# bacpop/sparrowhawk

Measured on AMD Instinct MI355X. Metric: Gbases/s assembled, k=31 150bp reads, higher is better.
Workload: dtype u64

## Files before the change

### sparrowhawk_amd/csrc/count_part.h

```cpp
#pragma once
#include <hip/hip_runtime.h>
#include <stdint.h>
#include <type_traits>
#include "kmer.h"

namespace shk {

static constexpr int PART_THREADS = 1024;
static constexpr int COUNT_THREADS = 1024;
static constexpr int PART_MAX_P = 16384;

struct PartParams {
    uint32_t P, G, slice_cap;
    int k, m;
    uint32_t max_n;
};

template <int RW> struct Rec { uint64_t w[RW]; };

__device__ __forceinline__ uint64_t sel4(uint32_t b, uint64_t t0, uint64_t t1, uint64_t t2, uint64_t t3) {
    uint64_t lo = (b & 1) ? t1 : t0;
    uint64_t hi = (b & 1) ? t3 : t2;
    return (b & 2) ? hi : lo;
}
// ... 871 lines not shown
        if (threadIdx.x == 0) ctl.prog_den = R ? R : 1u;
        for (uint32_t r0 = w_begin; r0 < w_end; r0 += 64) {
            if (ctl.overflow || ctl.n_used > (S / 10) * 9) { atomicMax(&ctl.prog_num, min(R, (r0 - w_begin) * (COUNT_THREADS / 64) + 1u)); break; }
            Rec<RW> rec = nxt;
            const uint32_t n = have_nxt ? (uint32_t)(rec.w[RW - 1] >> 58) + 1u : 0u;
            if (n) rec_canonicalise<RW>(rec.w, n, k);
            const uint32_t wgt = w_nxt;
            nxt = nxt2; have_nxt = have_nxt2; w_nxt = w_nxt2;
            have_nxt2 = fetch(r0 + 128u + (uint32_t)lane, nxt2, w_nxt2);
            if (n && !rec_insert<W>(tb.rt, ctl, rec, wgt)) {
                if (ovf && mod == 1 && (r0 - w_begin) * 2u < (w_end - w_begin)) ctl.overflow = 1;
                else expand(rec, n, wgt);
            }
        }
        {
            constexpr uint32_t SRc = decltype(tb.rt)::SR;
            auto &rt = tb.rt;
            if (threadIdx.x < 64) rt.nhist[threadIdx.x] = 0;
            __syncthreads();
            for (uint32_t s = threadIdx.x; s < SRc; s += COUNT_THREADS)
                if (rt.rst[s] >= 3u) atomicAdd(&rt.nhist[(uint32_t)(rt.w[s][RW - 1] >> 58)], 1u);
            __syncthreads();
            if (threadIdx.x < 64) {
                const uint32_t v = rt.nhist[threadIdx.x];
                uint32_t incl = v;
                for (int o = 1; o < 64; o <<= 1) { const uint32_t u = __shfl_up(incl, o); if (lane >= o) incl += u; }
                rt.nbase[threadIdx.x] = incl - v;
                if (threadIdx.x == 63) ctl.n_recs = incl;
            }
            __syncthreads();
            for (uint32_t s = threadIdx.x; s < SRc; s += COUNT_THREADS)
                if (rt.rst[s] >= 3u) rt.order[atomicAdd(&rt.nbase[(uint32_t)(rt.w[s][RW - 1] >> 58)], 1u)] = (uint16_t)s;
            __syncthreads();
            const uint32_t n_recs = ctl.n_recs;
            if (threadIdx.x == 0 && ctl.prog_num == 0) ctl.prog_den = n_recs ? n_recs : 1u;
            __syncthreads();
            for (uint32_t i = threadIdx.x; i < n_recs; i += COUNT_THREADS) {
                if (ctl.overflow || ctl.n_used > (S / 10) * 9) { atomicMax(&ctl.prog_num, i - threadIdx.x + 1u); break; }
                const uint32_t s = rt.order[i];
                Rec<RW> rec;
#pragma unroll
                for (int o = 0; o < RW; o++) rec.w[o] = rt.w[s][o];
                expand(rec, (uint32_t)(rec.w[RW - 1] >> 58) + 1u, rt.rst[s] - 2u);
            }
        }
        __syncthreads();
        const bool over = ctl.overflow != 0 || ctl.n_used > (S / 10) * 9;
        if (over && ovf && mod == 1) {
            defer(mine, true);
            return;
        }
        if (over) {
            if (mod >= 4096 || ctl.sp + 1 > 16) { if (threadIdx.x == 0) flags[0] = 1; break; }
            __syncthreads();
            if (threadIdx.x == 0) {
                const uint32_t num = ctl.prog_num ? ctl.prog_num : ctl.prog_den;
                const double est = (double)ctl.n_used * (double)ctl.prog_den / (double)num;
                uint32_t factor = 2;
                while ((double)factor * (0.6 * S) < est && mod * factor < 4096u) factor <<= 1;
                ctl.st_res[ctl.sp] = res; ctl.st_step[ctl.sp] = mod; ctl.st_factor[ctl.sp] = factor; ctl.st_next[ctl.sp] = 0;
                ctl.sp += 1;
            }
            continue;
        }
        static_assert(2u * decltype(tb.rt)::SR >= S, "emit list");
        table_emit<W>(tb, ctl, mine, threshold, histo, out_keys, out_cnt, out_cap, out_cursor, reinterpret_cast<uint16_t *>(tb.rt.rst), whist);
    }
    if (threadIdx.x == 0 && ovf && defer_after) atomicAdd(&ovf_n[1], 1u);
   }();
  }
    __syncthreads();
    for (uint32_t b = threadIdx.x; b < 500; b += COUNT_THREADS)
        if (whist[b]) atomicAdd(&histo[b], (unsigned long long)whist[b]);
    if (threadIdx.x == 0 && ctl.n_inst) atomicAdd(n_inst, ctl.n_inst);
}


template <int W> struct DedupeShared {
    RecTable<W, (W == 1 ? 3072u : ((69632u / (16u * W + 6u)) & ~63u))> rt;
};
template <int W>
__global__ __launch_bounds__(COUNT_THREADS, W <= 2 ? 8 : 4) void k_dedupe_partitions(
                                                                     RunView rvw, uint32_t p_first, uint32_t n_parts,
                                                                     const unsigned long long *__restrict__ base,
                                                                     uint64_t *__restrict__ out_recs, uint32_t *__restrict__ out_w,
                                                                     uint32_t *__restrict__ n_out, uint32_t *__restrict__ work_counter,
                                                                     OvfRec *__restrict__ ovf , uint32_t *__restrict__ ovf_n,
                                                                     uint32_t defer_after, uint32_t kmer_cap,
                                                                     uint32_t *__restrict__ verdict_out ) {
    constexpr int RW = 2 * W;
    __shared__ DedupeShared<W> tb;
    __shared__ CountCtl ctl;
    __shared__ uint32_t wtot[4];
    constexpr uint32_t SR = decltype(tb.rt)::SR;
    const int lane = threadIdx.x & 63;
    const int k = rvw.k;
    const uint32_t S_runs = rvw.S;
    const uint32_t n_here = n_parts - p_first;
    __shared__ uint32_t forced_sh;
    if (threadIdx.x == 0) forced_sh = 0;
    __syncthreads();
    bool forced = false;
    uint32_t pi_next = 0;
    for (uint32_t pi = blockIdx.x; pi < n_here; pi = pi_next) {
        const uint32_t p = p_first + pi;
        uint32_t f = 0; unsigned long long addr = 0;
        if (threadIdx.x < S_runs) { f = rvw.run_cnt[(uint64_t)p * S_runs + threadIdx.x]; addr = rvw.run_addr16[(uint64_t)p * S_runs + threadIdx.x]; }
        forced = forced_sh != 0;
        if (forced) {
            unsigned long long inst = 0;
            const uint64_t *src = reinterpret_cast<const uint64_t *>(addr << 4);
            for (uint32_t i = 0; i < f; i++) inst += (src[(uint64_t)i * RW + RW - 1] >> 58) + 1ull;
            __syncthreads();
            if (threadIdx.x == 0) { ctl.part_inst = 0; ctl.next_pi = gridDim.x + atomicAdd(work_counter, 1u); }
            __syncthreads();
            for (int o = 32; o > 0; o >>= 1) inst += __shfl_down(inst, o);
            if (lane == 0 && inst) atomicAdd(&ctl.part_inst, inst);
            __syncthreads();
            pi_next = ctl.next_pi;
            if (threadIdx.x == 0) {
                n_out[p] = 0;
                if (ctl.part_inst) { const uint32_t slot = atomicAdd(ovf_n, 1u); OvfRec o; o.p = p; o.est_distinct = 0u; o.instances = ctl.part_inst; ovf[slot] = o; }
            }
            continue;
        }
        uint32_t incl = f;
        if (threadIdx.x < 256) {
            for (int o = 1; o < 64; o <<= 1) { const uint32_t v = __shfl_up(incl, o); if (lane >= o) incl += v; }
            if (lane == 63) wtot[threadIdx.x >> 6] = incl;
        }
        __syncthreads();
        if (threadIdx.x < 256) {
            uint32_t off = 0;
            for (uint32_t w = 0; w < (threadIdx.x >> 6); w++) off += wtot[w];
            if (threadIdx.x < S_runs) { ctl.pre[threadIdx.x] = off + incl - f; ctl.roff[threadIdx.x] = addr; }
        }
        if (threadIdx.x == 0) {
            ctl.pre[S_runs] = wtot[0] + wtot[1] + wtot[2] + wtot[3];
            ctl.rec_used = 0; ctl.n_emit = 0; ctl.part_inst = 0;
            ctl.next_pi = gridDim.x + atomicAdd(work_counter, 1u);
        }
        for (uint32_t s = threadIdx.x; s < SR; s += COUNT_THREADS) tb.rt.rst[s] = 0;
        __syncthreads();
        pi_next = ctl.next_pi;
        const uint32_t R = ctl.pre[S_runs];
        auto hand_over = [&]() {
            unsigned long long inst = 0;
            const uint32_t pw = (((R + (COUNT_THREADS / 64) - 1) / (COUNT_THREADS / 64)) + 63u) & ~63u;
            const uint32_t wb = min(R, (threadIdx.x >> 6) * pw), we = min(R, wb + pw);
            uint32_t lo = 0, hi = S_runs;
            { const uint32_t r = min(wb + (uint32_t)lane, R ? R - 1u : 0u);
              while (hi - lo > 1) { const uint32_t mid = (lo + hi) >> 1; if (ctl.pre[mid] <= r) lo = mid; else hi = mid; } }
            uint32_t nx = ctl.pre[lo + 1];
            for (uint32_t r = wb + (uint32_t)lane; r < we; r += 64) {
                while (r >= nx) { lo++; nx = ctl.pre[lo + 1]; }
                const uint64_t *src = reinterpret_cast<const uint64_t *>(ctl.roff[lo] << 4) + (uint64_t)(r - ctl.pre[lo]) * RW;
                inst += (src[RW - 1] >> 58) + 1ull;
            }
            for (int o = 32; o > 0; o >>= 1) inst += __shfl_down(inst, o);
            if (lane == 0 && inst) atomicAdd(&ctl.part_inst, inst);
            __syncthreads();
            if (threadIdx.x == 0) {
                n_out[p] = 0;
                if (R) { const uint32_t slot = atomicAdd(ovf_n, 1u); OvfRec o; o.p = p; o.est_distinct = 0u; o.instances = ctl.part_inst; ovf[slot] = o; }
            }
        };
        uint64_t *dst = out_recs + base[p] * RW;
        uint32_t *dst_w = out_w + base[p];
        const uint32_t per_wave = (((R + (COUNT_THREADS / 64) - 1) / (COUNT_THREADS / 64)) + 63u) & ~63u;
        const uint32_t w_begin = min(R, (threadIdx.x >> 6) * per_wave), w_end = min(R, w_begin + per_wave);
        uint32_t run_lo = 0, run_next = 0;
        {
            uint32_t lo = 0, hi = S_runs;
            const uint32_t r = min(w_begin + (uint32_t)lane, R ? R - 1u : 0u);
            while (hi - lo > 1) { const uint32_t mid = (lo + hi) >> 1; if (ctl.pre[mid] <= r) lo = mid; else hi = mid; }
            run_lo = lo; run_next = ctl.pre[lo + 1];
        }
        auto fetch = [&](uint32_t r, Rec<RW> &rec) -> uint32_t {
            if (r >= w_end) return 0u;
            while (r >= run_next) { run_lo++; run_next = ctl.pre[run_lo + 1]; }
            const uint64_t *src = reinterpret_cast<const uint64_t *>(ctl.roff[run_lo] << 4) + (uint64_t)(r - ctl.pre[run_lo]) * RW;
#pragma unroll
            for (int o = 0; o < RW; o += 2) {
                const ulonglong2 v2 = *reinterpret_cast<const ulonglong2 *>(src + o);
                rec.w[o] = v2.x; rec.w[o + 1] = v2.y;
            }
            return 1u;
        };
        Rec<RW> nxt, nxt2;
#pragma unroll
        for (int o = 0; o < RW; o++) { nxt.w[o] = 0; nxt2.w[o] = 0; }
        uint32_t have_nxt = fetch(w_begin + (uint32_t)lane, nxt);
        uint32_t have_nxt2 = fetch(w_begin + 64u + (uint32_t)lane, nxt2);
        for (uint32_t r0 = w_begin; r0 < w_end; r0 += 64) {
            Rec<RW> rec = nxt;
            const uint32_t n = have_nxt ? (uint32_t)(rec.w[RW - 1] >> 58) + 1u : 0u;
            if (n) rec_canonicalise<RW>(rec.w, n, k);
            nxt = nxt2; have_nxt = have_nxt2;
            have_nxt2 = fetch(r0 + 128u + (uint32_t)lane, nxt2);
            const bool pass = n && !rec_insert<W>(tb.rt, ctl, rec);
            const unsigned long long m = __ballot(pass);
            if (m) {
                uint32_t at = 0;
                if (lane == (int)__builtin_ctzll(m)) at = atomicAdd(&ctl.n_emit, (uint32_t)__popcll(m));
                at = __shfl(at, (int)__builtin_ctzll(m)) + (uint32_t)__popcll(m & ((1ull << lane) - 1ull));
                if (pass) { part_store_record<RW>(rec.w, dst + (uint64_t)at * RW); dst_w[at] = 1u; }
            }
        }
        auto &rt = tb.rt;
        if (threadIdx.x < 64) rt.nhist[threadIdx.x] = 0;
        __syncthreads();
        for (uint32_t s = threadIdx.x; s < SR; s += COUNT_THREADS)
            if (rt.rst[s] >= 3u) atomicAdd(&rt.nhist[(uint32_t)(rt.w[s][RW - 1] >> 58)], 1u);
        __syncthreads();
        const uint32_t n_pass = ctl.n_emit;
        if (threadIdx.x < 64) {
            const uint32_t v = rt.nhist[threadIdx.x];
            uint32_t incl2 = v;
            for (int o = 1; o < 64; o <<= 1) { const uint32_t u = __shfl_up(incl2, o); if (lane >= o) incl2 += u; }
            rt.nbase[threadIdx.x] = n_pass + incl2 - v;
            if (threadIdx.x == 63) ctl.n_recs = n_pass + incl2;
        }
        __syncthreads();
        const bool hand = ovf && (ctl.n_recs > kmer_cap || (R > kmer_cap / 4u && 2u * ctl.n_recs > R));
        if (ovf && threadIdx.x == 0 && R) {
            const uint32_t add = hand ? 0x10001u : 1u;
            const uint32_t x = atomicAdd(&ovf_n[1], add) + add;
            const uint32_t n_over = x >> 16, n_tried = x & 0xFFFFu;
            if (defer_after && n_over >= defer_after && 2u * n_over >= n_tried) {
                forced_sh = 1u;
                if (verdict_out) atomicOr(verdict_out, 0x80000000u);
            }
        }
        if (hand) { hand_over(); continue; }
        for (uint32_t s = threadIdx.x; s < SR; s += COUNT_THREADS) {
            const uint32_t st = rt.rst[s];
            if (st < 3u) continue;
            const uint32_t at = atomicAdd(&rt.nbase[(uint32_t)(rt.w[s][RW - 1] >> 58)], 1u);
            uint64_t r[RW];
#pragma unroll
            for (int o = 0; o < RW; o++) r[o] = rt.w[s][o];
            part_store_record<RW>(r, dst + (uint64_t)at * RW);
            dst_w[at] = st - 2u;
        }
        __syncthreads();
        if (threadIdx.x == 0) n_out[p] = ctl.n_recs;
    }
}

template <int W>
__global__ __launch_bounds__(COUNT_THREADS, W <= 2 ? 8 : 4) void k_count_weighted(
    const uint64_t *__restrict__ recs, const uint32_t *__restrict__ weights, const unsigned long long *__restrict__ base,
    const uint32_t *__restrict__ n_recs, uint32_t p_first, uint32_t n_parts, uint32_t merge , int k, uint32_t threshold,
    unsigned long long *__restrict__ histo, KeyArr<W> out_keys, uint32_t *__restrict__ out_cnt,
    unsigned long long out_cap, unsigned long long *__restrict__ out_cursor,
    unsigned long long *__restrict__ n_inst, OvfRec *__restrict__ ovf, uint32_t *__restrict__ ovf_n,
    unsigned long long *__restrict__ work_and_tally ,
    uint32_t probe_groups, uint32_t defer_after,
    EmitRanges er ) {
    constexpr int RW = 2 * W;
    constexpr uint32_t S = KmerTable<W>::S;
    __shared__ KmerTable<W> tb;
    __shared__ CountCtlCore ctl;
    constexpr uint32_t ELIST = W == 1 ? S : 64;
    __shared__ uint16_t elist[ELIST];
    __shared__ uint32_t whist[500];
    __shared__ uint32_t next_g_sh, force_sh;
    const int lane = threadIdx.x & 63;
    for (uint32_t b = threadIdx.x; b < 500; b += COUNT_THREADS) whist[b] = 0;
    if (threadIdx.x == 0) ctl.n_inst = 0;
    const uint32_t n_groups = (n_parts + merge - 1) / merge;
    unsigned long long mine = 0;
    auto count_range = [&](const uint32_t (&pm)[4], uint32_t nm) -> bool {
        uint32_t Rj[4]; unsigned long long bj[4]; uint32_t Rt = 0;
#pragma unroll
        for (int j = 0; j < 4; j++) {
            const bool in = (uint32_t)j < nm;
            Rj[j] = in ? n_recs[pm[j]] : 0u; bj[j] = in ? base[pm[j]] : 0ull;
            Rt += Rj[j];
        }
        auto fetch = [&](uint32_t r, Rec<RW> &rec, uint32_t &wgt) {
            if (r < Rt) {
                unsigned long long at = bj[0] + r;
                uint32_t pre = Rj[0];
#pragma unroll
                for (int j = 1; j < 4; j++) { if (r >= pre) at = bj[j] + (r - pre); pre += Rj[j]; }
                const uint64_t *src = recs + at * RW;
#pragma unroll
                for (int o = 0; o < RW; o += 2) {
                    const ulonglong2 v2 = *reinterpret_cast<const ulonglong2 *>(src + o);
                    rec.w[o] = v2.x; rec.w[o + 1] = v2.y;
                }
                wgt = weights[at];
            }
        };
        Rec<RW> nxt; uint32_t w_nxt = 0;
#pragma unroll
        for (int o = 0; o < RW; o++) nxt.w[o] = 0;
        fetch(threadIdx.x, nxt, w_nxt);
        __syncthreads();
        if (threadIdx.x == 0) {
            ctl.n_used = 0; ctl.overflow = 0; ctl.n_emit = 0; ctl.wave_cursor = 0; ctl.rec_used = 0;
            ctl.prog_num = 0; ctl.prog_den = Rt ? Rt : 1u;
        }
        kmer_table_reset<W>(tb, ctl);
        mine = 0;
        for (uint32_t r0 = 0; r0 < Rt; r0 += COUNT_THREADS) {
            if (ctl.overflow || ctl.n_used > (S / 10) * 9) break;
            Rec<RW> rec = nxt; const uint32_t weight = w_nxt;
            const uint32_t r = r0 + threadIdx.x;
            fetch(r + COUNT_THREADS, nxt, w_nxt);
            if (r >= Rt) continue;
            const uint32_t n = (uint32_t)(rec.w[RW - 1] >> 58) + 1u;
            Kmer<W> f = km_zero<W>();
            for (uint32_t s = 0; s < n; s++) {
                if (ctl.overflow || ctl.n_used > (S / 10) * 9) break;
                if (s) {
#pragma unroll
                    for (int o = 0; o < RW - 1; o++) rec.w[o] = (rec.w[o] >> 2) | (rec.w[o + 1] << 62);
                    rec.w[RW - 1] >>= 2;
                }
                Kmer<W> rv;
#pragma unroll
                for (int j = 0; j < W; j++) rv.w[j] = ~rec.w[j];
                rv.w[W - 1] &= km_topmask<W>(k);
                if (s) km_push_back<W>(f, (uint32_t)(rec.w[W - 1] >> ((2 * (k - 1)) & 63)) & 3u, k);
                else f = km_revcomp<W>(rv, k);
                const bool use_r = km_less<W>(rv, f);
                Kmer<W> c;
#pragma unroll
                for (int j = 0; j < W; j++) c.w[j] = use_r ? rv.w[j] : f.w[j];
                const uint32_t h = km_mix32<W>(c);
                if (!lds_insert<W>(tb, ctl, c, h ^ __builtin_amdgcn_alignbit(h, h, 19), weight, true)) ctl.overflow = 1;
                mine += weight;
            }
        }
        __syncthreads();
        return !(ctl.overflow != 0 || ctl.n_used > (S / 10) * 9);
    };
    auto emit = [&](uint32_t er_g) {
        if constexpr (W == 1) table_emit<W>(tb, ctl, mine, threshold, histo, out_keys, out_cnt, out_cap, out_cursor, elist, whist, 0u, er, er_g);
        else table_emit<W>(tb, ctl, mine, threshold, histo, out_keys, out_cnt, out_cap, out_cursor, tb.state, whist, 0u, er, er_g);
    };
    auto mark_broken = [&]() { if (threadIdx.x == 0 && er.broken) *er.broken = 1u; };
    uint32_t *const tally = reinterpret_cast<uint32_t *>(work_and_tally) + 1;
    bool in_sample = true;
    auto defer = [&](uint32_t p, bool was_tried) {
        const uint32_t R = n_recs[p];
        const uint64_t *src = recs + base[p] * RW;
        const uint32_t *src_w = weights + base[p];
        mark_broken();
        __syncthreads();
        if (threadIdx.x == 0) { ctl.tried = 0; ctl.part_inst = 0; }
        __syncthreads();
        unsigned long long m = was_tried ? mine : 0ull;
        for (int o = 32; o > 0; o >>= 1) m += __shfl_down(m, o);
        if (lane == 0 && m) atomicAdd(&ctl.tried, m);
        unsigned long long inst = 0;
        for (uint32_t r = threadIdx.x; r < R; r += COUNT_THREADS)
            inst += ((src[(uint64_t)r * RW + RW - 1] >> 58) + 1ull) * (unsigned long long)src_w[r];
        for (int o = 32; o > 0; o >>= 1) inst += __shfl_down(inst, o);
        if (lane == 0 && inst) atomicAdd(&ctl.part_inst, inst);
        __syncthreads();
        if (threadIdx.x == 0 && R) {
            const double est = ctl.tried ? (double)ctl.n_used * (double)ctl.part_inst / (double)ctl.tried : (double)ctl.part_inst;
            const uint32_t slot = atomicAdd(ovf_n, 1u);
            OvfRec o; o.p = p; o.est_distinct = !was_tried ? 0u  : est > 4.0e9 ? 0xFFFFFFFFu : est < 1.0 ? 1u : (uint32_t)est; o.instances = ctl.part_inst;
            ovf[slot] = o;
        }
        if (threadIdx.x == 0 && was_tried && defer_after && in_sample) atomicAdd(tally, 0x10001u);
    };
    uint32_t g_next = 0;
    for (uint32_t g = blockIdx.x; g < n_groups; in_sample = false, g = g_next) {
        uint32_t pm[4] = {0, 0, 0, 0}, nm = 0;
#pragma unroll
        for (uint32_t j = 0; j < 4; j++) {
            const uint32_t pj = g + j * n_groups;
            const bool v = j < merge && pj < n_parts && pj >= p_first;
#pragma unroll
            for (uint32_t q = 0; q < 4; q++) if (v && nm == q) pm[q] = pj;
            nm += v ? 1u : 0u;
        }
        __syncthreads();
        if (threadIdx.x == 0) {
            const unsigned long long wt = atomicAdd(work_and_tally, 1ull);
            const uint32_t x = (uint32_t)(wt >> 32), n_over = x >> 16, n_tried = x & 0xFFFFu;
            next_g_sh = gridDim.x + (uint32_t)wt;
            force_sh = (defer_after && g >= probe_groups && n_over >= defer_after && 4u * n_over >= 3u * n_tried) ? 1u : 0u;
        }
        __syncthreads();
        g_next = next_g_sh;
        if (nm == 0) continue;
        if (force_sh) {
#pragma unroll
            for (uint32_t j = 0; j < 4; j++) if (j < nm) defer(pm[j], false);
            continue;
        }
        if (nm > 1 && count_range(pm, nm)) {
            emit(g);
            if (threadIdx.x == 0 && defer_after && in_sample) atomicAdd(tally, nm);
            continue;
        }
        if (nm > 1) mark_broken();
#pragma unroll
        for (uint32_t j = 0; j < 4; j++) {
            if (j >= nm) continue;
            const uint32_t one[4] = {pm[j], 0, 0, 0};
            if (count_range(one, 1u)) { emit(nm == 1 ? g : 0xFFFFFFFFu); if (threadIdx.x == 0 && defer_after && in_sample) atomicAdd(tally, 1u); }
            else defer(pm[j], true);
        }
    }
    __syncthreads();
    for (uint32_t b = threadIdx.x; b < 500; b += COUNT_THREADS)
        if (whist[b]) atomicAdd(&histo[b], (unsigned long long)whist[b]);
    if (threadIdx.x == 0 && ctl.n_inst) atomicAdd(n_inst, ctl.n_inst);
}

template <int RW>
__global__ __launch_bounds__(256) void k_pack_dedup(const uint64_t *__restrict__ src, const uint32_t *__restrict__ src_w,
                                                    const unsigned long long *__restrict__ src_base, const uint32_t *__restrict__ n_out,
                                                    const unsigned long long *__restrict__ dst_base,
                                                    uint64_t *__restrict__ dst, uint32_t *__restrict__ dst_w) {
    const uint32_t p = blockIdx.x, R = n_out[p];
    const uint64_t *sp = src + src_base[p] * RW;
    uint64_t *dp = dst + dst_base[p] * RW;
    for (uint32_t r = threadIdx.x; r < R; r += blockDim.x) {
#pragma unroll
        for (int o = 0; o < RW; o += 2)
            *reinterpret_cast<ulonglong2 *>(dp + (uint64_t)r * RW + o) = *reinterpret_cast<const ulonglong2 *>(sp + (uint64_t)r * RW + o);
        dst_w[dst_base[p] + r] = src_w[src_base[p] + r];
    }
}

// ... 267 lines not shown
```

### sparrowhawk_amd/csrc/ctl_words.h

```cpp
#pragma once
#include <stddef.h>
#include <stdint.h>

namespace shk {

static constexpr int CTL_WORDS = 32;

struct CountWords {
    union { unsigned long long row_cursor;
            unsigned long long g_instances; };
    union { unsigned long long instances;
            unsigned long long g_overflow; };
    uint32_t part_too_large, bucket_splits;
    uint32_t n_handed_over, tally;
    unsigned long long bucket_list_len;
    unsigned long long spare5[3];
    uint32_t p1_spare, p1_seg_too_long;
    union { unsigned long long p1_max_fill;
            unsigned long long bloom_keys; };
    unsigned long long spare10;
    unsigned long long probe_work;
    unsigned long long dedupe_work;
    unsigned long long spare13;
    uint32_t groups_out, group_tally;
    unsigned long long spare15[7];
    unsigned long long er_cursor;
    unsigned long long er_broken;
    unsigned long long spare24[8];
};
static inline unsigned tally_tried(uint32_t t) { return t & 0xFFFFu; }
static inline unsigned tally_over(uint32_t t) { return t >> 16; }
static inline unsigned long long er_rows(unsigned long long cursor) { return cursor >> 32; }

struct GraphWords {
    unsigned long long spare0;
    unsigned long long table_flag;
    unsigned long long slots_used;
    unsigned long long n_cand, n_tips;
    union { unsigned long long tips_removed;
            unsigned long long n_splitters; };
    union { unsigned long long bubbles_removed;
            unsigned long long n_chains; };
    unsigned long long n_ring_splitters;
    uint32_t collapse_flag, n_spl_wanted;
    unsigned long long n_alive;
    unsigned long long n_walked;
    unsigned long long spare11[2];
    union { unsigned long long xq_count;
            unsigned long long halflink_flags; };
    unsigned long long writer_flag;
    unsigned long long spare15;
    unsigned long long r0_tips_removed, r0_bubbles_removed;
    unsigned long long plan_state, plan_bytes, plan_emitted;
    unsigned long long spare21[11];
};

#define SHK_CTL_AT(S, m, slot, half) static_assert(offsetof(S, m) == (slot) * 8 + (half) * 4, #S "::" #m " moved")
static_assert(sizeof(CountWords) == CTL_WORDS * 8 && sizeof(GraphWords) == CTL_WORDS * 8, "32 control words");
SHK_CTL_AT(CountWords, row_cursor, 0, 0);     SHK_CTL_AT(CountWords, g_instances, 0, 0);
SHK_CTL_AT(CountWords, instances, 1, 0);      SHK_CTL_AT(CountWords, g_overflow, 1, 0);
SHK_CTL_AT(CountWords, part_too_large, 2, 0); SHK_CTL_AT(CountWords, bucket_splits, 2, 1);
SHK_CTL_AT(CountWords, n_handed_over, 3, 0);  SHK_CTL_AT(CountWords, tally, 3, 1);
SHK_CTL_AT(CountWords, bucket_list_len, 4, 0);
SHK_CTL_AT(CountWords, p1_spare, 8, 0);       SHK_CTL_AT(CountWords, p1_seg_too_long, 8, 1);
SHK_CTL_AT(CountWords, p1_max_fill, 9, 0);    SHK_CTL_AT(CountWords, bloom_keys, 9, 0);
SHK_CTL_AT(CountWords, probe_work, 11, 0);    SHK_CTL_AT(CountWords, dedupe_work, 12, 0);
SHK_CTL_AT(CountWords, groups_out, 14, 0);    SHK_CTL_AT(CountWords, group_tally, 14, 1);
SHK_CTL_AT(CountWords, er_cursor, 22, 0);     SHK_CTL_AT(CountWords, er_broken, 23, 0);
SHK_CTL_AT(GraphWords, spare0, 0, 0);         SHK_CTL_AT(GraphWords, table_flag, 1, 0);
SHK_CTL_AT(GraphWords, slots_used, 2, 0);     SHK_CTL_AT(GraphWords, n_cand, 3, 0);
SHK_CTL_AT(GraphWords, n_tips, 4, 0);
SHK_CTL_AT(GraphWords, tips_removed, 5, 0);   SHK_CTL_AT(GraphWords, n_splitters, 5, 0);
SHK_CTL_AT(GraphWords, bubbles_removed, 6, 0); SHK_CTL_AT(GraphWords, n_chains, 6, 0);
SHK_CTL_AT(GraphWords, n_ring_splitters, 7, 0);
SHK_CTL_AT(GraphWords, collapse_flag, 8, 0);  SHK_CTL_AT(GraphWords, n_spl_wanted, 8, 1);
SHK_CTL_AT(GraphWords, n_alive, 9, 0);        SHK_CTL_AT(GraphWords, n_walked, 10, 0);
SHK_CTL_AT(GraphWords, xq_count, 13, 0);      SHK_CTL_AT(GraphWords, halflink_flags, 13, 0);
SHK_CTL_AT(GraphWords, writer_flag, 14, 0);
SHK_CTL_AT(GraphWords, r0_tips_removed, 16, 0); SHK_CTL_AT(GraphWords, r0_bubbles_removed, 17, 0);
SHK_CTL_AT(GraphWords, plan_state, 18, 0);    SHK_CTL_AT(GraphWords, plan_bytes, 19, 0);
SHK_CTL_AT(GraphWords, plan_emitted, 20, 0);
#undef SHK_CTL_AT

}
```

### sparrowhawk_amd/csrc/pipeline.h

```cpp
#pragma once
#include <stdint.h>
#include <string>
#include <vector>
#include <map>
#include <memory>

namespace shk {

struct ShardComm;

class TextArrival {
public:
    virtual ~TextArrival() {}
    virtual const char *base() const = 0;
    virtual size_t total() const = 0;
    virtual void wait_range(size_t begin, size_t end) = 0;
    void wait_all() { wait_range(0, total()); }
    virtual int finish(std::string &err) = 0;
};

struct RawContig {
    const char *ext = nullptr; size_t ext_n = 0;
    std::string own;
    uint64_t kc = 0;
    const char *head = nullptr, *tail = nullptr; uint32_t ends_n = 0;
    const char *data() const { return ext ? ext : own.data(); }
    size_t size() const { return ext ? ext_n : own.size(); }
};

struct StageTimes {
    std::map<std::string, double> ms;
    void add(const std::string &k, double v) { ms[k] += v; }
};

struct DevPiece { const uint32_t *d_bases, *d_seg_off; uint64_t n_seg, n_bases; };

class IPipeline {
public:
    virtual ~IPipeline() {}
    virtual int count_batch(const uint32_t *d_bases, const uint32_t *d_seg_off, uint64_t n_seg,
                            uint64_t n_bases, std::string &err) = 0;
    virtual int count_batch_host(uint32_t *d_bases, uint32_t *d_seg_off, const uint32_t *h_bases, const uint32_t *h_seg_off,
                                 uint64_t n_seg, uint64_t n_bases, std::string &err) = 0;
    virtual int count_batch_pieces(const DevPiece *pieces, size_t n_pieces, std::string &err) = 0;
    virtual void expect_more_batches() = 0;
    virtual void set_bloom(bool on) = 0;
    virtual void set_verbose(bool on) = 0;
    virtual void single_batch_resident(bool on) = 0;
    virtual int histogram(uint64_t histo[500], uint32_t emit_threshold, std::string &err) = 0;
    virtual int filter(uint32_t threshold, std::string &err) = 0;
    virtual uint64_t total_instances() const = 0;
    virtual uint64_t n_distinct() const = 0;
    virtual uint64_t n_solid() const = 0;
    virtual int get_distinct(uint64_t *keys, uint32_t *counts, uint64_t cap, std::string &err) = 0;
    virtual int get_solid(uint64_t *keys, uint32_t *counts, uint64_t cap, std::string &err) = 0;
    virtual int build_graph(std::string &err) = 0;
    virtual int correct(bool tips, bool bubbles, std::string &err) = 0;
    virtual int collapse(std::vector<RawContig> &out, std::string &err, const char **json = nullptr, size_t *json_len = nullptr,
                         uint64_t *n_contigs = nullptr, TextArrival **arrival = nullptr) = 0;
    virtual int get_adjacency(uint8_t *adj_initial, uint8_t *adj_final, uint8_t *alive,
                              uint64_t cap, std::string &err) = 0;
    virtual int shard_partition(const uint32_t *d_bases, const uint32_t *d_seg_off, uint64_t n_seg, uint64_t n_bases,
                                uint32_t n_partitions, std::vector<uint64_t> &part_records, std::string &err) = 0;
    virtual uint32_t rec_words() const = 0;
    virtual int shard_pack(void *d_send, const uint64_t *base_records, uint32_t n_partitions, std::string &err) = 0;
    virtual int shard_dedupe(std::vector<uint64_t> &part_records, std::string &err) = 0;
    virtual int shard_pack_dedup(void *d_send, void *d_send_w, const uint64_t *base_records, uint32_t n_partitions, std::string &err) = 0;
    virtual void shard_drop_dedup() = 0;
    virtual int shard_count(const void *d_recv, const void *d_recv_w , const uint64_t *run_off, const uint32_t *run_cnt,
                            uint32_t n_owned, uint32_t n_sources, uint32_t emit_threshold, uint64_t histo[500], std::string &err) = 0;
    virtual int shard_rows(uint32_t threshold, const void **keys_soa, const void **cnt, uint64_t *n, std::string &err) = 0;
    virtual int shard_set_solid(const void *const *keys_soa, const void *cnt, uint64_t n, const uint64_t histo[500],
                                uint64_t total_instances, std::string &err) = 0;
    virtual int shard_keep_local(uint32_t world, uint32_t rank, uint32_t n_count_partitions, const uint64_t *rows_per_rank,
                                 const uint64_t histo[500], uint64_t total_instances, std::string &err) = 0;
    virtual bool sharded_graph() const = 0;
    virtual uint64_t n_solid_global() const = 0;
    virtual int shard_assemble(ShardComm *comm, bool tips, bool bubbles, std::vector<RawContig> &out, std::string &err) = 0;
    virtual StageTimes &times() = 0;
    virtual void drain() = 0;
    virtual void *stream() = 0;
    virtual int device() const = 0;
};

class DeferScope {
public:
    explicit DeferScope(IPipeline *pipe);
    ~DeferScope();
    DeferScope(const DeferScope &) = delete;
    DeferScope &operator=(const DeferScope &) = delete;
private:
    IPipeline *pipe_; void *list_; void *prev_;
};

IPipeline *make_pipeline(int k, std::string &err);
int device_count();
int current_device();
int set_device(int dev);

int host_canonical(const char *seq, uint32_t k, uint64_t *out_words, int *orient);
uint64_t host_nthash(const char *seq, uint32_t k);

int device_upload(const void *host, size_t bytes, void **dptr, std::string &err);
void device_free(void *dptr);
void device_pool_trim();
void *device_pool_alloc(size_t &bytes);
int stream_read_gbs(size_t bytes, int iters, double *gbs, std::string &err);
void device_pool_release(void *p, size_t bytes);
std::shared_ptr<void> mem_acct_new();
std::shared_ptr<void> mem_acct_set(std::shared_ptr<void> a);
uint64_t mem_acct_peak(const std::shared_ptr<void> &a);
uint64_t mem_acct_current(const std::shared_ptr<void> &a);
void mem_acct_replay(const int64_t *deltas, size_t n, uint64_t *peak, uint64_t *current);
int device_stream_sync(void *stream, std::string &err);
int device_copy_h2d_async(void *dst, const void *src, size_t bytes, void *stream, std::string &err);
int device_download(void *host, const void *dptr, size_t bytes, std::string &err);

}
```

### sparrowhawk_amd/csrc/pipeline.hip

```cpp
#include <hip/hip_runtime.h>
#include <hipcub/hipcub.hpp>
#include <thread>
#include <stdint.h>
#include <stdio.h>
#include <stdlib.h>
#include <string.h>
#include <algorithm>
#include <atomic>
#include <chrono>
#include <map>
#include <memory>
#include <mutex>
#include <string>
#include <vector>

#include "ctl_words.h"
#include "kmer.h"
#include "pipeline.h"
#include "shard_comm.h"
#include "unitig_graph.h"
#include "unitig_graph_gpu.h"

namespace shk {

// ... 203 lines not shown
}

static std::mutex g_stream_mu;
static std::multimap<int, hipStream_t> &stream_cache() { static auto *c = new std::multimap<int, hipStream_t>(); return *c; }
static hipStream_t stream_pool_get(int dev) {
    std::lock_guard<std::mutex> lk(g_stream_mu);
    auto it = stream_cache().find(dev);
    if (it == stream_cache().end()) return nullptr;
    hipStream_t s = it->second; stream_cache().erase(it); return s;
}
static void stream_pool_put(int dev, hipStream_t s) {
    {
        std::lock_guard<std::mutex> lk(g_stream_mu);
        if (stream_cache().size() < 32) { stream_cache().emplace(dev, s); return; }
    }
    (void)hipStreamDestroy(s);
}

static std::mutex &upload_token(int dev) { static std::mutex m[16]; return m[(unsigned)dev % 16u]; }

static inline int grid_for(uint64_t work, int block = 256, int max_blocks = 256 * 16) {
    uint64_t b = (work + block - 1) / block;
    if (b < 1) b = 1;
    if (b > (uint64_t)max_blocks) b = max_blocks;
    return (int)b;
}

static inline hipError_t stream_wait(hipStream_t s) {
    static const bool blocking = getenv("SHK_BLOCKING_SYNC") != nullptr;
    if (blocking) return hipStreamSynchronize(s);
    const auto t0 = std::chrono::steady_clock::now();
    for (;;) {
        const hipError_t e = hipStreamQuery(s);
        if (e != hipErrorNotReady) return e;
        if (std::chrono::steady_clock::now() - t0 > std::chrono::milliseconds(5)) return hipStreamSynchronize(s);
    }
}

struct EvTimer {
    hipEvent_t a, b; hipStream_t st; bool ok = false;
    explicit EvTimer(hipStream_t s, bool on = true) : st(s) {
        if (!on) return;
        ok = hipEventCreate(&a) == hipSuccess && hipEventCreate(&b) == hipSuccess;
        if (ok) (void)hipEventRecord(a, st);
    }
    bool on() const { return ok; }
    double stop() {
        if (!ok) return 0.0;
        (void)hipEventRecord(b, st); (void)hipEventSynchronize(b);
        float ms = 0; (void)hipEventElapsedTime(&ms, a, b);
        return ms;
    }
    ~EvTimer() { if (ok) { (void)hipEventDestroy(a); (void)hipEventDestroy(b); } }
    void mark() { if (ok) (void)hipEventRecord(b, st); }
    double elapsed() {
        if (!ok) return 0.0;
        (void)hipEventSynchronize(b);
        float ms = 0; (void)hipEventElapsedTime(&ms, a, b);
        return ms;
    }
    struct Pending { std::string name; hipEvent_t a, b; };
    void stop_later(const char *name, std::vector<Pending> &pending) {
        if (!ok) return;
        (void)hipEventRecord(b, st);
        pending.push_back(Pending{name, a, b});
        ok = false;
    }
    static void resolve(std::vector<Pending> &pending, StageTimes &times) {
        for (auto &p : pending) {
            (void)hipEventSynchronize(p.b);
            float ms = 0; (void)hipEventElapsedTime(&ms, p.a, p.b);
            times.add(p.name, ms);
            (void)hipEventDestroy(p.a); (void)hipEventDestroy(p.b);
        }
        pending.clear();
    }
};

static inline uint64_t env_u64(const char *name, uint64_t dflt) {
    const char *v = getenv(name);
    return (v && *v) ? strtoull(v, nullptr, 10) : dflt;
}

__global__ __launch_bounds__(256) void k_fill2(uint32_t *a, unsigned long long na, uint32_t va, uint32_t *b, unsigned long long nb, uint32_t vb) {
    const unsigned long long stride = (unsigned long long)gridDim.x * blockDim.x;
    for (unsigned long long i = (unsigned long long)blockIdx.x * blockDim.x + threadIdx.x; i < na + nb; i += stride) {
        if (i < na) a[i] = va; else b[i - na] = vb;
    }
}
__global__ __launch_bounds__(256) void k_stride_fill(unsigned long long *out, uint32_t n, unsigned long long stride) {
    for (uint32_t i = blockIdx.x * blockDim.x + threadIdx.x; i < n; i += gridDim.x * blockDim.x) out[i] = (unsigned long long)i * stride;
}
static inline hipError_t fill2_async(void *a, size_t bytes_a, uint32_t va, void *b, size_t bytes_b, uint32_t vb, hipStream_t st) {
    const unsigned long long na = bytes_a / 4, nb = bytes_b / 4;
    const unsigned long long blocks = std::min<unsigned long long>((na + nb + 255) / 256, 2048ull);
    if (!blocks) return hipSuccess;
    hipLaunchKernelGGL(k_fill2, dim3((uint32_t)blocks), dim3(256), 0, st, (uint32_t *)a, na, va, (uint32_t *)b, nb, vb);
    return hipGetLastError();
}

static constexpr uint32_t ARRIVAL_SLAB = 64u << 10;
__global__ __launch_bounds__(256) void k_text_to_host(const char *__restrict__ src, char *__restrict__ dst_host, unsigned long long bytes,
                                                      uint32_t n_slabs, uint32_t *__restrict__ flags_host) {
    for (uint32_t s = blockIdx.x; s < n_slabs; s += gridDim.x) {
        const unsigned long long o = (unsigned long long)s * ARRIVAL_SLAB;
        const uint32_t m = (uint32_t)(bytes - o < ARRIVAL_SLAB ? bytes - o : ARRIVAL_SLAB);
        const uint4 *a = reinterpret_cast<const uint4 *>(src + o);
        uint4 *d = reinterpret_cast<uint4 *>(dst_host + o);
        const uint32_t nv = m >> 4;
#pragma unroll 4
        for (uint32_t i = threadIdx.x; i < nv; i += 256) d[i] = a[i];
        if (threadIdx.x < (m & 15u)) dst_host[o + (nv << 4) + threadIdx.x] = src[o + (nv << 4) + threadIdx.x];
        __threadfence_system();
        __syncthreads();
        if (threadIdx.x == 0) __hip_atomic_store(&flags_host[s], 1u, __ATOMIC_RELEASE, __HIP_MEMORY_SCOPE_SYSTEM);
    }
}
__global__ __launch_bounds__(1024) void k_ends_to_host(const char *__restrict__ text, const unsigned long long *__restrict__ src ,
                                                       uint32_t nc, uint32_t E, char *__restrict__ ends_host, uint32_t *__restrict__ flag_host) {
    const unsigned long long total = (unsigned long long)nc * 2ull * E;
    for (unsigned long long t = threadIdx.x; t < total; t += blockDim.x) {
        const uint32_t c = (uint32_t)(t / (2ull * E)), r = (uint32_t)(t % (2ull * E)), side = r / E, j = r % E;
        const unsigned long long off = src[2 * c], len = src[2 * c + 1];
        const unsigned long long m = len < E ? len : (unsigned long long)E;
        char ch = 0;
        if (j < m) ch = side ? text[off + len - m + j] : text[off + j];
        ends_host[t] = ch;
    }
    __threadfence_system();
    __syncthreads();
    if (threadIdx.x == 0) __hip_atomic_store(flag_host, 1u, __ATOMIC_RELEASE, __HIP_MEMORY_SCOPE_SYSTEM);
}
__global__ __launch_bounds__(256) void k_text_to_host_planned(const char *__restrict__ src, char *__restrict__ dst_host,
                                                              const unsigned long long *__restrict__ plan) {
    if (plan[0] != 1ull) return;
    const unsigned long long bytes = plan[1];
    const unsigned long long nv = bytes >> 4;
    const uint4 *a = reinterpret_cast<const uint4 *>(src);
    uint4 *d = reinterpret_cast<uint4 *>(dst_host);
    for (unsigned long long i = (unsigned long long)blockIdx.x * 256u + threadIdx.x; i < nv; i += (unsigned long long)gridDim.x * 256u) d[i] = a[i];
    if (blockIdx.x == 0 && threadIdx.x < (bytes & 15ull)) dst_host[(nv << 4) + threadIdx.x] = src[(nv << 4) + threadIdx.x];
}
class SlabArrival : public TextArrival {
public:
    void set(char *dst, size_t bytes, volatile uint32_t *flags, uint32_t n_slabs, hipStream_t st) { base_ = dst; total_ = bytes; flags_ = flags; n_slabs_ = n_slabs; st_ = st; failed_.store(false); }
    const char *base() const override { return base_; }
    size_t total() const override { return total_; }
    static bool spin_until(volatile uint32_t *f, std::atomic<bool> &failed) {
        if (__atomic_load_n(f, __ATOMIC_ACQUIRE)) return true;
        const auto t0 = std::chrono::steady_clock::now();
        for (uint32_t it = 0;; it++) {
            if (__atomic_load_n(f, __ATOMIC_ACQUIRE)) return true;
            if (failed.load(std::memory_order_relaxed)) return false;
            if ((it & 0xFFFu) == 0xFFFu && std::chrono::steady_clock::now() - t0 > std::chrono::seconds(20)) { failed.store(true); return false; }
            __builtin_ia32_pause();
        }
    }
    void wait_range(size_t begin, size_t end) override {
        if (end > total_) end = total_;
        if (begin >= end) return;
        for (size_t s = begin / ARRIVAL_SLAB; s <= (end - 1) / ARRIVAL_SLAB; s++) if (!spin_until(flags_ + s, failed_)) return;
    }
    int finish(std::string &err) override {
        const hipError_t e = hipStreamSynchronize(st_);
        if (e != hipSuccess || failed_.load()) { err = std::string("download of the contigs failed") + (e != hipSuccess ? std::string(": ") + hipGetErrorString(e) : std::string()); return -5; }
        return 0;
    }
    std::atomic<bool> failed_{false};
private:
    char *base_ = nullptr; size_t total_ = 0; volatile uint32_t *flags_ = nullptr; uint32_t n_slabs_ = 0; hipStream_t st_ = nullptr;
};

static inline int part_win(int k) {
    static const int forced = [] { const char *e = getenv("SHK_PART_WIN"); return e ? atoi(e) : 0; }();
    if (k < 23) return 8;
    if (k < 31) return 16;
    if (forced == 16 || forced == 18 || forced == 20) return forced;
    return k <= 32 ? 18 : 16;
}
static inline int part_m(int k) { return k - part_win(k) + 1; }

template <int W> class Pipeline : public IPipeline {
public:
    explicit Pipeline(int k) : k_(k) {}
    ~Pipeline() override {
        drain();
        EvTimer::resolve(pending_timers_, times_);
        if (copy_stream_) { (void)hipStreamSynchronize(copy_stream_); stream_pool_put(stream_dev_ + 1000, copy_stream_); }
        if (stream_) stream_pool_put(stream_dev_, stream_);
    }
    int init(std::string &err) {
        HIPCHK(hipGetDevice(&stream_dev_));
        { int cus = 0; (void)hipDeviceGetAttribute(&cus, hipDeviceAttributeMultiprocessorCount, stream_dev_); n_cus_ = cus > 0 ? cus : 256; }
        stream_ = stream_pool_get(stream_dev_);
        if (!stream_) HIPCHK(hipStreamCreate(&stream_));
        HIPCHK(ctl_.alloc(CTL_WORDS, err) ? hipErrorOutOfMemory : hipSuccess);
        if (mbox_.alloc(MBOX_BYTES, err)) return -4;
        return 0;
    }
    StageTimes &times() override { EvTimer::resolve(pending_timers_, times_); return times_; }
    void drain() override {
        if (copy_stream_) (void)hipStreamSynchronize(copy_stream_);
        if (!stream_) return;
        std::string e;
        if (wd_comm_) (void)comm_stream_wait(wd_comm_, stream_, e);
        else (void)hipStreamSynchronize(stream_);
    }
    void *stream() override { return (void *)stream_; }
    int device() const override { return stream_dev_; }
    uint64_t total_instances() const override { return total_instances_; }
    uint64_t n_distinct() const override { return n_distinct_; }
    uint64_t n_solid() const override { return n_solid_; }

    int alloc_table(uint64_t slots, std::string &err) {
        for (int j = 0; j < W; j++) if (int rc = tkeys_[j].alloc(slots, err)) return rc;
        if (int rc = tcnt_.alloc(slots, err)) return rc;
        if (W > 1) if (int rc = tstate_.alloc(slots, err)) return rc;
        tslots_ = slots;
        if (W == 1) HIPCHK(hipMemsetAsync(tkeys_[0].p, 0xFF, slots * 8, stream_));
        else HIPCHK(hipMemsetAsync(tstate_.p, 0, slots * 4, stream_));
        HIPCHK(hipMemsetAsync(tcnt_.p, 0, slots * 4, stream_));
        return 0;
    }
    CountTable<W> table_view() {
        CountTable<W> t;
        for (int j = 0; j < W; j++) t.keys.w[j] = tkeys_[j].p;
        t.cnt = tcnt_.p; t.state = tstate_.p; t.mask = tslots_ - 1;
        return t;
    }

    int count_batch_global(const uint32_t *d_bases, const uint32_t *d_seg_off, uint64_t n_seg,
                           uint64_t n_bases, std::string &err) {
        if (n_seg >= 0xFFFFFFFFull || n_bases >= 0xFFFFFFFFull) { err = "batch too large (>= 2^32 bases)"; return -1; }
        if (n_seg == 0) return 0;
        const uint64_t inst_ub = n_bases - n_seg * (uint64_t)(k_ - 1);
        if (tslots_ == 0) {
            uint64_t want = inst_ub / 4 + 1024;
            uint64_t slots = 1ull << 16;
            while (slots < want) slots <<= 1;
            if (int rc = alloc_table(slots, err)) return rc;
            pending_.clear();
        }
        pending_.push_back({d_bases, d_seg_off, n_seg});
        for (;;) {
            HIPCHK(hipMemsetAsync(ctl_.p, 0, sizeof(CountWords), stream_));
            EvTimer t(stream_);
            hipLaunchKernelGGL(k_count_segments<W>, dim3(grid_for(n_seg)), dim3(256), 0, stream_, d_bases,
                               d_seg_off, (uint32_t)n_seg, k_, table_view(), (uint32_t *)ctl(&CountWords::g_overflow),
                               ctl(&CountWords::g_instances));
            HIPCHK(hipGetLastError());
            double ms = t.stop();
            CountWords h;
            HIPCHK(fetch_ctl(&h, &CountWords::g_instances, &CountWords::g_overflow));
            WAIT_STREAM();
            if ((uint32_t)h.g_overflow == 0) {
                times_.add("count_kernel", ms);
                total_instances_ += h.g_instances;
                return 0;
            }
            if (pending_.size() > 1) { err = "count table overflow across batches"; return -6; }
            times_.add("count_retry", ms);
            if (int rc = alloc_table(tslots_ * 4, err)) return rc;
        }
    }

    template <int WBLK, int NBLK>
    void launch_partition_t(const uint32_t *d_bases, const uint32_t *d_seg_off, uint32_t n_seg) {
        hipLaunchKernelGGL((k_partition<W, WBLK, NBLK>), dim3(pp_.G), dim3(PART_THREADS), 0, stream_, d_bases, d_seg_off,
                           n_seg, pp_, recs_.p, fill_.p, ctl(&CountWords::p1_spare));
    }
    void launch_partition(int win, const uint32_t *d_bases, const uint32_t *d_seg_off, uint32_t n_seg) {
        if (win == 20) launch_partition_t<10, 2>(d_bases, d_seg_off, n_seg);
        else if (win == 18) launch_partition_t<9, 2>(d_bases, d_seg_off, n_seg);
        else if (win == 16) launch_partition_t<16, 1>(d_bases, d_seg_off, n_seg);
        else launch_partition_t<8, 1>(d_bases, d_seg_off, n_seg);
    }

    int count_batch(const uint32_t *d_bases, const uint32_t *d_seg_off, uint64_t n_seg, uint64_t n_bases,
                    std::string &err) override {
        return count_batch_impl(d_bases, d_seg_off, nullptr, nullptr, n_seg, n_bases, err);
    }
    int count_batch_host(uint32_t *d_bases, uint32_t *d_seg_off, const uint32_t *h_bases, const uint32_t *h_seg_off,
                         uint64_t n_seg, uint64_t n_bases, std::string &err) override {
        return count_batch_impl(d_bases, d_seg_off, h_bases, h_seg_off, n_seg, n_bases, err);
    }
    int count_batch_pieces(const DevPiece *pieces, size_t n_pieces, std::string &err) override {
        std::vector<DevPiece> list;
        uint64_t n_seg = 0, n_bases = 0;
        for (size_t i = 0; i < n_pieces; i++)
            if (pieces[i].n_seg) { list.push_back(pieces[i]); n_seg += pieces[i].n_seg; n_bases += pieces[i].n_bases; }
        if (list.empty()) return 0;
        if (list.size() == 1) return count_batch_impl(list[0].d_bases, list[0].d_seg_off, nullptr, nullptr, n_seg, n_bases, err);
        if (global_mode_) {
            for (const DevPiece &pc : list)
                if (int rc = count_batch_impl(pc.d_bases, pc.d_seg_off, nullptr, nullptr, pc.n_seg, pc.n_bases, err)) return rc;
            return 0;
        }
        piece_list_ = std::move(list);
        struct Clear { std::vector<DevPiece> &v; ~Clear() { v.clear(); } } clear{piece_list_};
        return count_batch_impl(piece_list_[0].d_bases, piece_list_[0].d_seg_off, nullptr, nullptr, n_seg, n_bases, err);
    }
    void launch_partition_all(int wblk, const uint32_t *d_bases, const uint32_t *d_seg_off, uint64_t n_seg) {
        if (piece_list_.empty()) { launch_partition(wblk, d_bases, d_seg_off, (uint32_t)n_seg); return; }
        for (const DevPiece &pc : piece_list_) launch_partition(wblk, pc.d_bases, pc.d_seg_off, (uint32_t)pc.n_seg);
    }
    int count_batch_impl(const uint32_t *d_bases, const uint32_t *d_seg_off, const uint32_t *h_bases, const uint32_t *h_seg_off,
                         uint64_t n_seg, uint64_t n_bases, std::string &err) {
        if (h_bases && (global_mode_ || n_seg == 0)) {
            HIPCHK(hipMemcpyAsync((void *)d_bases, h_bases, ((n_bases + 15) / 16 + 1) * 4, hipMemcpyHostToDevice, stream_));
            HIPCHK(hipMemcpyAsync((void *)d_seg_off, h_seg_off, (n_seg + 1) * 4, hipMemcpyHostToDevice, stream_));
            h_bases = nullptr;
        }
        if (global_mode_) return count_batch_global(d_bases, d_seg_off, n_seg, n_bases, err);
        if (n_seg >= 0xFFFFFFFFull || n_bases >= 0xFFFFFFFFull) { err = "batch too large (>= 2^32 bases)"; return -1; }
        if (n_seg == 0) return 0;
        if (have_parts_) if (int rc = pack_current_batch(err)) return rc;
        constexpr int RW = 2 * W;
        const int wblk = part_win(k_);
        const uint64_t inst_ub = n_bases - n_seg * (uint64_t)(k_ - 1);
        const int cus = n_cus_;
        const uint64_t n_super = (n_seg + PART_THREADS - 1) / PART_THREADS;
        pp_.k = k_; pp_.m = k_ - wblk + 1;
        pp_.max_n = std::min<uint32_t>(32u * RW - 3u - (uint32_t)(k_ - 1), 63u);
        if (uint64_t mn = env_u64("SHK_PART_MAXN", 0)) pp_.max_n = std::min<uint32_t>(pp_.max_n, (uint32_t)mn);
        pp_.G = (uint32_t)std::min<uint64_t>((uint64_t)std::min(cus, 256), n_super);
        if (uint64_t fg = env_u64("SHK_PART_G", 0)) pp_.G = (uint32_t)std::min<uint64_t>(pp_.G, fg);
        uint32_t P = 64;
        const uint64_t per_part = env_u64("SHK_PART_INST", W == 1 ? 100000 : 40000);
        while (P < (uint32_t)PART_MAX_P && (uint64_t)P * per_part < inst_ub) P <<= 1;
        if (uint64_t fp = env_u64("SHK_PART_P", 0)) P = (uint32_t)fp;
        if (forced_P_) P = forced_P_;
        if (!batches_.empty()) P = pp_.P;
        pp_.P = P;
        const uint64_t per_rec = pp_.max_n >= 16 ? 4 : 2;
        uint64_t cap = inst_ub / (per_rec * P * pp_.G) + 32 + env_u64("SHK_SLICE_PAD", 0);
        if (cap_override_) { cap = cap_override_; cap_override_ = 0; }
        for (int attempt = 0; attempt < 2; attempt++) {
            if (env_u64("SHK_SLICE_NOSKEW", 0) == 0)
                while ((cap * RW * 8) % 2048 < 256 || (cap * RW * 8) % 2048 > 1792) cap++;
            if (cap * pp_.G > 0xFFFFFFF0ull) { err = "a partition would hold more than 2^32 records"; return -1; }
            pp_.slice_cap = (uint32_t)cap;
            const uint64_t n_slices = (uint64_t)P * pp_.G;
            if (int rc = recs_.alloc(n_slices * cap * RW, err)) return rc;
            if (int rc = fill_.alloc(n_slices, err)) return rc;
            HIPCHK(fill2_async(fill_.p, n_slices * 4, 0u, ctl_.p, sizeof(CountWords), 0u, stream_));
            EvTimer t(stream_);
            if (h_bases && attempt == 0) {
                uint64_t C = env_u64("SHK_H2D_PIECES", 4);
                if (C < 1) C = 1;
                while (C > 1 && n_seg / C < (uint64_t)PART_THREADS * pp_.G) C--;
                if (!copy_stream_) copy_stream_ = stream_pool_get(stream_dev_ + 1000);
                if (!copy_stream_) HIPCHK(hipStreamCreateWithFlags(&copy_stream_, hipStreamNonBlocking));
                const uint64_t n_words = (n_bases + 15) / 16 + 1;
                std::vector<hipEvent_t> evs((size_t)C, nullptr);
                struct EvGuard { std::vector<hipEvent_t> &v; ~EvGuard() { for (auto e : v) if (e) (void)hipEventDestroy(e); } } evg{evs};
                struct CopyDrain { hipStream_t s; std::unique_lock<std::mutex> token; ~CopyDrain() { (void)hipStreamSynchronize(s); } }
                    copy_drain{copy_stream_, std::unique_lock<std::mutex>(upload_token(stream_dev_))};
                for (uint64_t c = 0; c < C; c++) {
                    const uint64_t s0 = n_seg * c / C, s1 = n_seg * (c + 1) / C;
                    const uint64_t w0 = h_seg_off[s0] >> 4, w1 = std::min<uint64_t>(n_words, (((uint64_t)h_seg_off[s1] + 15) >> 4) + 1);
                    HIPCHK(hipMemcpyAsync((void *)(d_seg_off + s0), h_seg_off + s0, (s1 - s0 + 1) * 4, hipMemcpyHostToDevice, copy_stream_));
                    HIPCHK(hipMemcpyAsync((void *)(d_bases + w0), h_bases + w0, (w1 - w0) * 4, hipMemcpyHostToDevice, copy_stream_));
                    HIPCHK(hipEventCreateWithFlags(&evs[c], hipEventDisableTiming));
                    HIPCHK(hipEventRecord(evs[c], copy_stream_));
                    HIPCHK(hipStreamWaitEvent(stream_, evs[c], 0));
                    launch_partition(wblk, d_bases, d_seg_off + s0, (uint32_t)(s1 - s0));
                }
                HIPCHK(hipGetLastError());
                times_.add("h2d_pieces_x1", (double)C);
                if (defer_p1_ && batches_.empty()) {
                    HIPCHK(fetch_ctl(mb_p1(), &CountWords::p1_spare, &CountWords::p1_max_fill));
                    t.stop_later("partition_with_upload", pending_timers_);
                    p1_ = P1Pending{true, d_bases, d_seg_off, n_seg, n_bases, cap};
                    return finish_partition(n_slices, err);
                }
                t.mark();
                CountWords h;
                HIPCHK(fetch_ctl(&h, &CountWords::p1_spare, &CountWords::p1_max_fill));
                WAIT_STREAM();
                if (h.p1_seg_too_long) { err = "a read segment exceeds 32768 bases (split it on the host)"; return -1; }
                if ((uint32_t)h.p1_max_fill <= cap) {
                    times_.add("partition_with_upload", t.elapsed());
                    if (int rc = finish_partition(n_slices, err)) return rc;
                    return 0;
                }
                times_.add("partition_retry", t.elapsed());
                cap = (uint64_t)(uint32_t)h.p1_max_fill + 8;
                continue;
            }
            launch_partition_all(wblk, d_bases, d_seg_off, n_seg);
            HIPCHK(hipGetLastError());
            if (defer_p1_ && attempt == 0 && batches_.empty() && piece_list_.empty()) {
                HIPCHK(fetch_ctl(mb_p1(), &CountWords::p1_spare, &CountWords::p1_max_fill));
                t.stop_later("partition_kernel", pending_timers_);
                p1_ = P1Pending{true, d_bases, d_seg_off, n_seg, n_bases, cap};
                return finish_partition(n_slices, err);
            }
            t.mark();
            CountWords h;
            HIPCHK(fetch_ctl(&h, &CountWords::p1_spare, &CountWords::p1_max_fill));
            WAIT_STREAM();
            const double ms = t.elapsed();
            if (h.p1_seg_too_long) { err = "a read segment exceeds 32768 bases (split it on the host)"; return -1; }
            const uint32_t max_fill = (uint32_t)h.p1_max_fill;
            if (max_fill <= cap) {
                times_.add("partition_kernel", ms);
                if (int rc = finish_partition(n_slices, err)) return rc;
                return 0;
            }
            times_.add("partition_retry", ms);
            cap = (uint64_t)max_fill + 8;
        }
        err = "partition slices overflowed twice";
        return -6;
    }

    int finish_partition(uint64_t n_slices, std::string &err) {
        constexpr int RW = 2 * W;
        have_parts_ = true;
        if (int rc = run_off_.alloc(n_slices, err)) return rc;
        if (int rc = run_cnt_.alloc(n_slices, err)) return rc;
        hipLaunchKernelGGL(k_make_runs, dim3(grid_for(n_slices)), dim3(256), 0, stream_, fill_.p, pp_, recs_.p,
                           (uint32_t)RW, run_off_.p, run_cnt_.p);
        HIPCHK(hipGetLastError());
        run_view_.run_addr16 = run_off_.p; run_view_.run_cnt = run_cnt_.p;
        run_view_.S = pp_.G; run_view_.k = k_; n_count_parts_ = pp_.P;
        return 0;
    }

    struct BatchRecs { DevBuf<uint64_t> dense; std::vector<unsigned long long> part_off;  };

    int pack_current_batch(std::string &err) {
        constexpr int RW = 2 * W;
        DevBuf<unsigned long long> tot, base;
        if (int rc = tot.alloc(pp_.P, err)) return rc;
        if (int rc = base.alloc(pp_.P, err)) return rc;
        hipLaunchKernelGGL(k_part_totals, dim3(pp_.P), dim3(256), 0, stream_, fill_.p, pp_, tot.p);
        HIPCHK(hipGetLastError());
        std::vector<unsigned long long> h(pp_.P);
        HIPCHK(hipMemcpyAsync(h.data(), tot.p, (size_t)pp_.P * 8, hipMemcpyDeviceToHost, stream_));
        WAIT_STREAM();
        std::unique_ptr<BatchRecs> b(new BatchRecs());
        b->part_off.assign(pp_.P + 1, 0);
        for (uint32_t p = 0; p < pp_.P; p++) b->part_off[p + 1] = b->part_off[p] + h[p];
        if (int rc = b->dense.alloc(b->part_off[pp_.P] * RW + 2, err)) return rc;
        HIPCHK(hipMemcpyAsync(base.p, b->part_off.data(), (size_t)pp_.P * 8, hipMemcpyHostToDevice, stream_));
        EvTimer t(stream_, stage_timers_);
        hipLaunchKernelGGL((k_pack_partition<2 * W>), dim3(pp_.P), dim3(256), 0, stream_, recs_.p, fill_.p, pp_, base.p, b->dense.p);
        HIPCHK(hipGetLastError());
        if (t.on()) times_.add("batch_pack_kernel", t.stop());
        WAIT_STREAM();
        batches_.push_back(std::move(b));
        recs_.release(); fill_.release(); run_off_.release(); run_cnt_.release(); have_parts_ = false;
        if (batches_.size() >= env_u64("SHK_MERGE_BATCHES_AT", 192)) return merge_batches(err);
        return 0;
    }

    int merge_batches(std::string &err) {
        constexpr int RW = 2 * W;
        if (batches_.size() < 2) return 0;
        if (int rc = make_batch_run_view(err)) return rc;
        std::unique_ptr<BatchRecs> m(new BatchRecs());
        m->part_off.assign(pp_.P + 1, 0);
        for (uint32_t p = 0; p < pp_.P; p++) {
            unsigned long long tot = 0;
            for (auto &b : batches_) tot += b->part_off[p + 1] - b->part_off[p];
            m->part_off[p + 1] = m->part_off[p] + tot;
        }
        if (int rc = m->dense.alloc(m->part_off[pp_.P] * RW + 2, err)) return rc;
        DevBuf<unsigned long long> base;
        if (int rc = base.alloc(pp_.P, err)) return rc;
        HIPCHK(hipMemcpyAsync(base.p, m->part_off.data(), (size_t)pp_.P * 8, hipMemcpyHostToDevice, stream_));
        EvTimer t(stream_);
        hipLaunchKernelGGL((k_merge_runs<RW>), dim3(pp_.P), dim3(256), 0, stream_, run_view_, base.p, m->dense.p);
        HIPCHK(hipGetLastError());
        if (t.on()) times_.add("batch_merge_kernel", t.stop());
        WAIT_STREAM();
        batches_.clear();
        batches_.push_back(std::move(m));
        run_off_.release(); run_cnt_.release(); have_parts_ = false;
        return 0;
    }

    int make_batch_run_view(std::string &err) {
        const uint32_t nb = (uint32_t)batches_.size();
        if (nb > 256) { err = "more than 256 batches per handle"; return -1; }
        const uint64_t n_runs = (uint64_t)pp_.P * nb;
        std::vector<unsigned long long> addr16(n_runs); std::vector<uint32_t> cnt(n_runs);
        for (uint32_t p = 0; p < pp_.P; p++) {
            unsigned long long r = 0;
            for (uint32_t b = 0; b < nb; b++) r += batches_[b]->part_off[p + 1] - batches_[b]->part_off[p];
            if (r > 0xFFFFFFF0ull) { err = "a partition holds more than 2^32 records"; return -1; }
        }
        for (uint32_t p = 0; p < pp_.P; p++)
            for (uint32_t b = 0; b < nb; b++) {
                const BatchRecs &B = *batches_[b];
                const unsigned long long c = B.part_off[p + 1] - B.part_off[p];
                if (c > 0xFFFFFFFFull) { err = "partition too large in one batch"; return -1; }
                addr16[(uint64_t)p * nb + b] = ((unsigned long long)(uintptr_t)B.dense.p >> 4) + B.part_off[p] * (unsigned long long)W;
                cnt[(uint64_t)p * nb + b] = (uint32_t)c;
            }
        if (int rc = run_off_.alloc(n_runs, err)) return rc;
        if (int rc = run_cnt_.alloc(n_runs, err)) return rc;
        HIPCHK(hipMemcpyAsync(run_off_.p, addr16.data(), n_runs * 8, hipMemcpyHostToDevice, stream_));
        HIPCHK(hipMemcpyAsync(run_cnt_.p, cnt.data(), n_runs * 4, hipMemcpyHostToDevice, stream_));
        WAIT_STREAM();
        run_view_.run_addr16 = run_off_.p; run_view_.run_cnt = run_cnt_.p;
        run_view_.S = nb; run_view_.k = k_; n_count_parts_ = pp_.P;
        have_parts_ = true;
        return 0;
    }
    void set_bloom(bool on) override { bloom_ = on; }
    void set_verbose(bool on) override { if (on) { stage_timers_ = true; keep_stages_ = true; } }
    void single_batch_resident(bool on) override { defer_p1_ = on && !global_mode_; }
    void expect_more_batches() override { if (!forced_P_ && batches_.empty() && !have_parts_) forced_P_ = (uint32_t)PART_MAX_P; }

    int run_count_partitions(const RunView &rv, uint32_t n_parts, uint32_t threshold, DevBuf<uint64_t> (&keys)[W],
                             DevBuf<uint32_t> &cnt, uint64_t &n_rows, uint64_t hist_out[500], uint64_t &inst_out,
                             uint64_t cap_hint, double &ms_out, std::string &err) {
        if (n_parts == 0) { n_rows = 0; inst_out = 0; memset(hist_out, 0, 500 * 8); ms_out = 0; return 0; }
        constexpr uint32_t S = CountShared<W>::S;
        const bool repartition = env_u64("SHK_NO_REPARTITION", 0) == 0 && rv.weights == nullptr;
        DevBuf<unsigned long long> dh;
        DevBuf<OvfRec> d_ovf; DevBuf<OvfItem> d_items; DevBuf<uint32_t> d_fill, d_list, d_maxfill, d_new; DevBuf<uint64_t> d_kmers; DevBuf<BucketRef> d_blist; DevBuf<unsigned long long> d_sumfill;
        const bool bloom = bloom_ && !bloom_off_once_;
        unsigned long long bloom_new = 0, bloom_kmer_bytes = 0, bloom_kmer_bytes_exact = 0;
        if (int rc = dh.alloc(500, err)) return rc;
        if (repartition) if (int rc = d_ovf.alloc(n_parts, err)) return rc;
        const bool split = W <= 2 && repartition && !bloom && rv.weights == nullptr && split_ready_ && split_base_.size() == n_parts && split_total_ > 0 &&
                           env_u64("SHK_COUNT_SPLIT", 1) != 0;
        struct DropSplit { Pipeline<W> *me; bool on; ~DropSplit() { if (on) me->shard_drop_dedup(); } } drop_split{this, split};
        uint64_t cap = cap_hint;
        for (int attempt = 0; attempt < (bloom ? 4 : 2); attempt++) {
            bloom_new = 0; bloom_kmer_bytes = 0; bloom_kmer_bytes_exact = 0;
            for (int j = 0; j < W; j++) if (int rc = keys[j].alloc(cap, err)) return rc;
            if (int rc = cnt.alloc(cap, err)) return rc;
            HIPCHK(fill2_async(dh.p, 500 * 8, 0u, ctl_.p, sizeof(CountWords), 0u, stream_));
            KeyArr<W> ok; for (int j = 0; j < W; j++) ok.w[j] = keys[j].p;
            const uint32_t probe_parts = (uint32_t)env_u64("SHK_PROBE_PARTS", 512);
            const uint32_t n_probe = (repartition && probe_parts && n_parts / 4 >= probe_parts) ? probe_parts : 0u;
            EvTimer t(stream_);
            if (split) {
                if (int rc = dd_base_.alloc(n_parts, err)) return rc;
                if (int rc = dd_n_.alloc(n_parts, err)) return rc;
                if (int rc = dd_recs_.alloc(split_total_ * 2 * W + 2, err)) return rc;
                if (int rc = dd_w_.alloc(split_total_ + 2, err)) return rc;
                if (split_stride_) {
                    hipLaunchKernelGGL(k_stride_fill, dim3((n_parts + 255) / 256), dim3(256), 0, stream_, dd_base_.p, n_parts, split_stride_);
                    HIPCHK(hipGetLastError());
                } else HIPCHK(hipMemcpyAsync(dd_base_.p, split_base_.data(), (size_t)n_parts * 8, hipMemcpyHostToDevice, stream_));
                const uint32_t defer_after = n_probe / 8;
                EvTimer t_a(stream_, stage_timers_);
                hipLaunchKernelGGL(k_dedupe_partitions<W>, dim3(std::min<uint32_t>(n_parts, 2u * (uint32_t)n_cus_)), dim3(COUNT_THREADS), 0, stream_,
                                   rv, 0u, n_parts, dd_base_.p, dd_recs_.p, dd_w_.p, dd_n_.p, (uint32_t *)ctl(&CountWords::dedupe_work),
                                   d_ovf.p, ctl(&CountWords::n_handed_over), defer_after, (S / 10) * 9, ctl(&CountWords::group_tally));
                HIPCHK(hipGetLastError());
                if (attempt == 0) t_a.stop_later("count_dedupe_kernel", pending_timers_);
                const uint32_t per_cu = 2u;
                uint32_t merge = (uint32_t)std::min<uint64_t>(std::max<uint64_t>(env_u64("SHK_COUNT_MERGE", 1), 1), 4);
                if (merge == 3) merge = 2;
                while (merge > 1 && (n_parts % merge != 0 || (n_parts / merge) % 256u != 0 || n_parts / merge < 2u * per_cu * (uint32_t)n_cus_)) merge >>= 1;
                const uint32_t n_groups = (n_parts + merge - 1) / merge;
                EmitRanges er{};
                er_groups_ = 0;
                if (n_parts % merge == 0 && (n_groups & (n_groups - 1u)) == 0 && n_groups <= GP_MAX && cap < (1ull << 28) &&
                    env_u64("SHK_GRAPH_RANGES", 1) != 0) {
                    if (int rc = er_off_.alloc(n_groups, err)) return rc;
                    if (int rc = er_msk_.alloc(n_groups, err)) return rc;
                    if (int rc = er_start_.alloc(n_groups, err)) return rc;
                    if (int rc = er_cnt_.alloc(n_groups, err)) return rc;
                    er.tab_cursor = ctl(&CountWords::er_cursor); er.broken = (uint32_t *)ctl(&CountWords::er_broken);
                    er.off = er_off_.p; er.msk = er_msk_.p; er.start = er_start_.p; er.cnt = er_cnt_.p;
                    er_groups_ = n_groups;
                }
                hipLaunchKernelGGL(k_count_weighted<W>, dim3(std::min<uint32_t>(n_groups, per_cu * (uint32_t)n_cus_)), dim3(COUNT_THREADS), 0, stream_,
                                   dd_recs_.p, dd_w_.p, dd_base_.p, dd_n_.p, 0u, n_parts, merge, rv.k, threshold, dh.p, ok, cnt.p, (unsigned long long)cap,
                                   ctl(&CountWords::row_cursor), ctl(&CountWords::instances), d_ovf.p, ctl(&CountWords::n_handed_over),
                                   (unsigned long long *)ctl(&CountWords::groups_out), 0u, defer_after, er);
            } else {
                auto kern = rv.weights ? k_count_partitions<W, true> : k_count_partitions<W, false>;
                hipLaunchKernelGGL(kern, dim3(std::min<uint32_t>(n_parts, (uint32_t)n_cus_)), dim3(COUNT_THREADS), 0, stream_, rv, n_parts, threshold,
                                   dh.p, ok, cnt.p, (unsigned long long)cap, ctl(&CountWords::row_cursor), ctl(&CountWords::instances),
                                   ctl(&CountWords::part_too_large), (const uint32_t *)nullptr, repartition ? d_ovf.p : (OvfRec *)nullptr,
                                   ctl(&CountWords::n_handed_over), (uint32_t *)ctl(&CountWords::probe_work), n_probe / 2, n_probe / 8);
            }
            HIPCHK(hipGetLastError());
            t.mark();
            CountWords h{};
            HIPCHK(fetch_ctl(&h, &CountWords::row_cursor, &CountWords::tally));
            HIPCHK(hipMemcpyAsync(hist_out, dh.p, 500 * 8, hipMemcpyDeviceToHost, stream_));
            if (split && er_groups_) HIPCHK(fetch_ctl(&h, &CountWords::er_cursor, &CountWords::er_broken));
            WAIT_STREAM();
            ms_out = t.elapsed();
            const uint32_t n_ovf = h.n_handed_over;
            if (env_u64("SHK_VERBOSE_TALLY", 0)) fprintf(stderr, "[shk] pass 2: %u partitions, %u handed over, tally tried %u / over %u, split %d\n", n_parts, n_ovf,
                                                    tally_tried(h.tally), tally_over(h.tally), (int)split);
            rows_scattered_ = (uint64_t)n_ovf * 4u > n_parts;
            if (n_ovf) {
                EvTimer t2(stream_);
                std::vector<OvfRec> ov(n_ovf);
                HIPCHK(hipMemcpy(ov.data(), d_ovf.p, (size_t)n_ovf * sizeof(OvfRec), hipMemcpyDeviceToHost));
                std::vector<OvfItem> items;
                items.reserve(n_ovf);
                std::vector<uint32_t> bad;
                uint32_t n_untried = 0;
                const unsigned long long fill_pct = env_u64("SHK_OVF_FILL_PCT", 110), cap_pct = env_u64("SHK_OVF_CAP_PCT", bloom ? 100 : 150);
                for (uint32_t i = 0; i < n_ovf; i++) {
                    if (ov[i].instances >= 0xFFFFFFF0ull) { bad.push_back(ov[i].p); continue; }
                    items.emplace_back();
                    OvfItem &item = items.back();
                    const unsigned long long per = (unsigned long long)S * fill_pct / 100;
                    const uint32_t F = (uint32_t)std::min<unsigned long long>(std::max<unsigned long long>((ov[i].instances + per - 1) / per, 2ull), OVF_MAX_F);
                    if (ov[i].est_distinct == 0) n_untried++;
                    const unsigned long long capb = ov[i].instances * cap_pct / (100ull * F) + 256;
                    item.p = ov[i].p; item.F = F; item.cap = (uint32_t)std::min<unsigned long long>(capb, 0xFFFFFFF0ull);
                    item.pad = 0; item.base = 0;
                }
                size_t n_good_total = 0;
                const int max_passes = (int)env_u64("SHK_OVF_MAX_PASSES", 4);
                for (int pass = 0; pass < max_passes && !items.empty(); pass++) {
                    const uint32_t ni = (uint32_t)items.size();
                    unsigned long long tot = 0;
                    for (auto &it : items) { it.base = tot; tot += (unsigned long long)it.F * it.cap; }
                    if (int rc = d_items.alloc(ni, err)) return rc;
                    if (int rc = d_fill.alloc((size_t)ni * OVF_MAX_F, err)) return rc;
                    if (int rc = d_kmers.alloc(tot * W, err)) return rc;
                    HIPCHK(hipMemcpyAsync(d_items.p, items.data(), (size_t)ni * sizeof(OvfItem), hipMemcpyHostToDevice, stream_));
                    if (bloom) {
                        if (int rc = d_new.alloc(ni, err)) return rc;
                        hipLaunchKernelGGL((k_ovf_scatter<W, true>), dim3(ni), dim3(COUNT_THREADS), 0, stream_, rv, d_items.p, d_kmers.p, d_fill.p, d_new.p);
                    } else {
                        hipLaunchKernelGGL((k_ovf_scatter<W, false>), dim3(ni), dim3(COUNT_THREADS), 0, stream_, rv, d_items.p, d_kmers.p, d_fill.p, (uint32_t *)nullptr);
                    }
                    HIPCHK(hipGetLastError());
                    if (int rc = d_maxfill.alloc(ni, err)) return rc;
                    unsigned long long n_buckets_ub = 0;
                    for (auto &it : items) n_buckets_ub += it.F;
                    if (int rc = d_blist.alloc(n_buckets_ub, err)) return rc;
                    HIPCHK(fill2_async(ctl(&CountWords::bucket_list_len), ctl_span(&CountWords::bucket_list_len), 0u, nullptr, 0, 0u, stream_));
                    if (int rc = d_sumfill.alloc(ni, err)) return rc;
                    hipLaunchKernelGGL(k_ovf_check, dim3(grid_for(ni)), dim3(256), 0, stream_, d_items.p, d_fill.p, ni, d_maxfill.p,
                                       d_blist.p, (uint32_t *)ctl(&CountWords::bucket_list_len), d_sumfill.p);
                    HIPCHK(hipGetLastError());
                    std::vector<uint32_t> mxf(ni), newc(bloom ? ni : 0);
                    std::vector<unsigned long long> smf(ni);
                    HIPCHK(hipMemcpyAsync(smf.data(), d_sumfill.p, (size_t)ni * 8, hipMemcpyDeviceToHost, stream_));
                    if (bloom) HIPCHK(hipMemcpyAsync(newc.data(), d_new.p, (size_t)ni * 4, hipMemcpyDeviceToHost, stream_));
                    HIPCHK(hipMemcpyAsync(mxf.data(), d_maxfill.p, (size_t)ni * 4, hipMemcpyDeviceToHost, stream_));
                    HIPCHK(fetch_ctl(&h, &CountWords::bucket_list_len, &CountWords::bucket_list_len));
                    WAIT_STREAM();
                    std::vector<OvfItem> again;
                    uint32_t n_good = 0;
                    for (uint32_t i = 0; i < ni; i++) {
                        if (mxf[i] <= items[i].cap) {
                            n_good++;
                            if (bloom) {
                                bloom_new += newc[i];
                                bloom_kmer_bytes += smf[i] * 8ull * W;
                            }
                        }
                        else if (pass + 1 < max_passes && (unsigned long long)mxf[i] + 256 < 0xFFFFFFF0ull) {
                            OvfItem it = items[i]; it.cap = mxf[i] + 256; again.push_back(it);
                        } else bad.push_back(items[i].p);
                    }
                    if (const uint32_t n_list = (uint32_t)h.bucket_list_len) {
                        const uint32_t bgrid = (uint32_t)std::min<unsigned long long>(h.bucket_list_len, 2ull * (unsigned long long)n_cus_);
                        hipLaunchKernelGGL(k_count_buckets<W>, dim3(bgrid), dim3(COUNT_THREADS), 0, stream_,
                                           d_blist.p, n_list, d_kmers.p, threshold, dh.p, ok, cnt.p, (unsigned long long)cap,
                                           ctl(&CountWords::row_cursor), ctl(&CountWords::instances), ctl(&CountWords::part_too_large), bloom ? 1u : 0u, ctl(&CountWords::bloom_keys));
                        HIPCHK(hipGetLastError());
                        WAIT_STREAM();
                    }
                    n_good_total += n_good;
                    items.swap(again);
                }
                if (!bad.empty()) {
                    if (int rc = d_list.alloc(bad.size(), err)) return rc;
                    HIPCHK(hipMemcpyAsync(d_list.p, bad.data(), bad.size() * 4, hipMemcpyHostToDevice, stream_));
                    hipLaunchKernelGGL(k_count_partitions<W>, dim3(std::min<uint32_t>((uint32_t)bad.size(), (uint32_t)n_cus_)), dim3(COUNT_THREADS), 0, stream_, rv, (uint32_t)bad.size(), threshold,
                                       dh.p, ok, cnt.p, (unsigned long long)cap, ctl(&CountWords::row_cursor), ctl(&CountWords::instances),
                                       ctl(&CountWords::part_too_large), (const uint32_t *)d_list.p, (OvfRec *)nullptr, (uint32_t *)nullptr, (uint32_t *)ctl(&CountWords::dedupe_work), 0u, 0u);
                    HIPCHK(hipGetLastError());
                }
                ms_out += t2.stop();
                times_.add("count_repartitioned_x1", (double)n_good_total);
                times_.add("count_deferred_untried_x1", (double)n_untried);
                times_.add("count_residue_rerun_x1", (double)bad.size());
                HIPCHK(fetch_ctl(&h, &CountWords::row_cursor, &CountWords::tally));
                HIPCHK(hipMemcpyAsync(hist_out, dh.p, 500 * 8, hipMemcpyDeviceToHost, stream_));
                WAIT_STREAM();
                times_.add("count_bucket_splits_x1", (double)h.bucket_splits);
                if (bloom) {
                    unsigned long long n_keys = 0;
                    HIPCHK(hipMemcpy(&n_keys, ctl(&CountWords::bloom_keys), ctl_span(&CountWords::bloom_keys), hipMemcpyDeviceToHost));
                    const unsigned long long singles = bloom_new > n_keys ? bloom_new - n_keys : 0ull;
                    hist_out[0] += singles;
                    h.instances += bloom_new;
                    for (uint32_t i = 0; i < n_ovf; i++) bloom_kmer_bytes_exact += ov[i].instances * 8ull * W;
                    times_.add("bloom_new_kmers_x1e-6", (double)bloom_new * 1e-6);
                    times_.add("bloom_singletons_never_stored_x1e-6", (double)singles * 1e-6);
                    times_.add("bloom_kmer_instances_MB_written", (double)bloom_kmer_bytes / 1e6);
                    times_.add("bloom_kmer_instances_MB_without_filter", (double)bloom_kmer_bytes_exact / 1e6);
                }
            }
            if (h.part_too_large) { err = "partition too large for the LDS table even after 4096-way residue splitting"; return -6; }
            n_rows = h.row_cursor; inst_out = h.instances;
            er_ok_ = split && er_groups_ && (uint32_t)h.er_broken == 0u && n_ovf == 0 && er_rows(h.er_cursor) == h.row_cursor;
            er_rows_ = n_rows;
            if (n_rows <= cap) {
                return 0;
            }
            cap = bloom ? n_rows + n_rows / 16 + 4096 : n_rows;
        }
        err = "row buffer overflowed twice";
        return -6;
    }

    int histogram(uint64_t histo[500], uint32_t emit_threshold, std::string &err) override {
        er_ok_ = false;
        if (!global_mode_) {
            memset(histo, 0, 500 * 8);
            n_distinct_ = 0; n_emitted_ = 0; emit_threshold_ = emit_threshold;
            if (!batches_.empty()) {
                if (have_parts_ && recs_.p) if (int rc = pack_current_batch(err)) return rc;
                if (int rc = make_batch_run_view(err)) return rc;
            }
            if (have_parts_) {
                const uint64_t inst_ub_rows = total_rows_hint();
                double ms = 0; uint64_t inst = 0;
                split_base_.assign(n_count_parts_, 0); split_total_ = 0; split_stride_ = 0;
                if (batches_.empty()) {
                    split_stride_ = (unsigned long long)pp_.G * pp_.slice_cap;
                    for (uint32_t p = 0; p < n_count_parts_; p++) split_base_[p] = (unsigned long long)p * pp_.G * pp_.slice_cap;
                    split_total_ = (unsigned long long)n_count_parts_ * pp_.G * pp_.slice_cap;
                } else {
                    for (uint32_t p = 0; p < n_count_parts_; p++) {
                        split_base_[p] = split_total_;
                        for (auto &b : batches_) split_total_ += b->part_off[p + 1] - b->part_off[p];
                    }
                }
                split_ready_ = true;
                int rc_p2 = run_count_partitions(run_view_, n_count_parts_, emit_threshold, ekeys_, ecnt_, n_emitted_, histo, inst,
                                                 inst_ub_rows, ms, err);
                if (p1_.on) {
                    if (rc_p2) { std::string e2; (void)e2; (void)hipStreamSynchronize(stream_); }
                    p1_.on = false;
                    const CountWords &h = *mb_p1();
                    if (h.p1_seg_too_long) { split_ready_ = false; err = "a read segment exceeds 32768 bases (split it on the host)"; return -1; }
                    if ((uint32_t)h.p1_max_fill > p1_.cap) {
                        times_.add("partition_retry", 1.0);
                        cap_override_ = (uint64_t)(uint32_t)h.p1_max_fill + 8;
                        have_parts_ = false; split_ready_ = false;
                        const bool d = defer_p1_; defer_p1_ = false;
                        const int rc1 = count_batch_impl(p1_.d_bases, p1_.d_seg_off, nullptr, nullptr, p1_.n_seg, p1_.n_bases, err);
                        defer_p1_ = d;
                        if (rc1) return rc1;
                        return histogram(histo, emit_threshold, err);
                    }
                }
                if (rc_p2) { split_ready_ = false; return rc_p2; }
                split_ready_ = false;
                times_.add("count_kernel", ms);
                total_instances_ = inst;
            }
            for (int i = 0; i < 500; i++) { histo_[i] = histo[i]; n_distinct_ += histo[i]; }
            return 0;
        }
        DevBuf<unsigned long long> dh;
        if (int rc = dh.alloc(500, err)) return rc;
        HIPCHK(hipMemsetAsync(dh.p, 0, 500 * 8, stream_));
        if (tslots_) {
            EvTimer t(stream_, stage_timers_);
            hipLaunchKernelGGL(k_histogram<W>, dim3(grid_for(tslots_)), dim3(256), 0, stream_, table_view(),
                               tslots_, dh.p);
            HIPCHK(hipGetLastError());
            if (t.on()) times_.add("histogram_kernel", t.stop());
        }
        HIPCHK(hipMemcpyAsync(histo, dh.p, 500 * 8, hipMemcpyDeviceToHost, stream_));
        WAIT_STREAM();
        n_distinct_ = 0;
        for (int i = 0; i < 500; i++) { histo_[i] = histo[i]; n_distinct_ += histo[i]; }
        return 0;
    }

    uint64_t total_rows_hint() const {
        uint64_t slots = (uint64_t)pp_.P * pp_.G * pp_.slice_cap;
        if (!batches_.empty()) { slots = 0; for (auto &b : batches_) slots += b->part_off[pp_.P]; }
        return std::max<uint64_t>(1u << 16, slots / 8);
    }

    int compact_into(uint32_t threshold, uint64_t expect, DevBuf<uint64_t> (&keys)[W], DevBuf<uint32_t> &cnt,
                     std::string &err) {
        for (int j = 0; j < W; j++) if (int rc = keys[j].alloc(expect, err)) return rc;
        if (int rc = cnt.alloc(expect, err)) return rc;
        if (!tslots_ || !expect) return 0;
        HIPCHK(hipMemsetAsync(ctl_.p, 0, sizeof(CountWords), stream_));
        KeyArr<W> ok; for (int j = 0; j < W; j++) ok.w[j] = keys[j].p;
        hipLaunchKernelGGL(k_compact<W>, dim3(grid_for(tslots_)), dim3(256), 0, stream_, table_view(), tslots_,
                           threshold, ok, cnt.p, ctl(&CountWords::row_cursor));
        HIPCHK(hipGetLastError());
        unsigned long long got = 0;
        HIPCHK(hipMemcpyAsync(&got, ctl(&CountWords::row_cursor), ctl_span(&CountWords::row_cursor), hipMemcpyDeviceToHost, stream_));
        WAIT_STREAM();
        if (got != expect) { err = "compaction count mismatch"; return -6; }
        return 0;
    }

    int filter(uint32_t threshold, std::string &err) override {
        uint64_t expect = 0;
        if (threshold >= 500) { err = "threshold out of range"; return -1; }
        for (uint32_t c = 1; c <= 500; c++) if (c > threshold) expect += histo_[c - 1];
        if (expect >= 0x7FFFFFFFull) { err = "too many solid k-mers for 32-bit node ids"; return -1; }
        EvTimer t(stream_, stage_timers_);
        if (global_mode_) {
            if (int rc = compact_into(threshold, expect, skeys_, scnt_, err)) return rc;
        } else if (threshold == emit_threshold_ || n_emitted_ == 0) {
            if (n_emitted_ != expect && threshold == emit_threshold_) { err = "emitted row count disagrees with the histogram"; return -6; }
            for (int j = 0; j < W; j++) skeys_[j].swap(ekeys_[j]);
            scnt_.swap(ecnt_);
            for (int j = 0; j < W; j++) ekeys_[j].release();
            ecnt_.release();
        } else {
            if (threshold < emit_threshold_) { err = "filter threshold below the emit threshold"; return -6; }
            er_ok_ = false;
            for (int j = 0; j < W; j++) if (int rc = skeys_[j].alloc(expect, err)) return rc;
            if (int rc = scnt_.alloc(expect, err)) return rc;
            HIPCHK(hipMemsetAsync(ctl_.p, 0, sizeof(CountWords), stream_));
            KeyArr<W> ik, ok;
            for (int j = 0; j < W; j++) { ik.w[j] = ekeys_[j].p; ok.w[j] = skeys_[j].p; }
            hipLaunchKernelGGL(k_compact_rows<W>, dim3(grid_for(n_emitted_)), dim3(256), 0, stream_, ik, ecnt_.p,
                               n_emitted_, threshold, ok, scnt_.p, ctl(&CountWords::row_cursor));
            HIPCHK(hipGetLastError());
            unsigned long long got = 0;
            HIPCHK(hipMemcpyAsync(&got, ctl(&CountWords::row_cursor), ctl_span(&CountWords::row_cursor), hipMemcpyDeviceToHost, stream_));
// ... 13 lines not shown
        std::vector<uint64_t> tmp(n ? n : 1);
        for (int j = 0; j < W; j++) {
            if (n) HIPCHK(hipMemcpy(tmp.data(), keys[j].p, n * 8, hipMemcpyDeviceToHost));
            for (uint64_t i = 0; i < n; i++) hk[i * W + j] = tmp[i];
        }
        if (n) HIPCHK(hipMemcpy(hc, cnt.p, n * 4, hipMemcpyDeviceToHost));
        return 0;
    }

    int get_distinct(uint64_t *keys, uint32_t *counts, uint64_t cap, std::string &err) override {
        if (cap < n_distinct_) { err = "buffer too small"; return -1; }
        DevBuf<uint64_t> dk[W]; DevBuf<uint32_t> dc;
        if (global_mode_) {
            if (int rc = compact_into(0, n_distinct_, dk, dc, err)) return rc;
        } else if (n_distinct_) {
            if (!have_parts_ || (!recs_.p && batches_.empty())) { err = "partition buffers already released"; return -2; }
            uint64_t rows = 0, hist[500], inst = 0; double ms = 0;
            bloom_off_once_ = true;
            const int rc = run_count_partitions(run_view_, n_count_parts_, 0, dk, dc, rows, hist, inst, n_distinct_, ms, err);
            bloom_off_once_ = false;
            if (rc) return rc;
            if (bloom_) { if (cap < rows) { err = "buffer too small"; return -1; } return copy_out(dk, dc, rows, keys, counts, err); }
            if (rows != n_distinct_) { err = "distinct row count mismatch"; return -6; }
        }
        return copy_out(dk, dc, n_distinct_, keys, counts, err);
    }
    int get_solid(uint64_t *keys, uint32_t *counts, uint64_t cap, std::string &err) override {
        if (cap < n_solid_) { err = "buffer too small"; return -1; }
        return copy_out(skeys_, scnt_, n_solid_, keys, counts, err);
    }

    int shard_partition(const uint32_t *d_bases, const uint32_t *d_seg_off, uint64_t n_seg, uint64_t n_bases,
                        uint32_t n_partitions, std::vector<uint64_t> &part_records, std::string &err) override {
        if (global_mode_) { err = "shard layer needs the partitioned counting mode"; return -1; }
        if (n_partitions < 1 || n_partitions > (uint32_t)PART_MAX_P || (n_partitions & (n_partitions - 1))) {
            err = "n_partitions must be a power of two <= 16384"; return -1;
        }
        forced_P_ = n_partitions;
        part_records.assign(n_partitions, 0);
        if (int rc = count_batch(d_bases, d_seg_off, n_seg, n_bases, err)) return rc;
        if (!have_parts_) return 0;
        DevBuf<unsigned long long> tot;
        if (int rc = tot.alloc(pp_.P, err)) return rc;
        hipLaunchKernelGGL(k_part_totals, dim3(pp_.P), dim3(256), 0, stream_, fill_.p, pp_, tot.p);
        HIPCHK(hipGetLastError());
        std::vector<unsigned long long> h(pp_.P);
        HIPCHK(hipMemcpyAsync(h.data(), tot.p, (size_t)pp_.P * 8, hipMemcpyDeviceToHost, stream_));
        WAIT_STREAM();
        for (uint32_t p = 0; p < pp_.P; p++) part_records[p] = h[p];
        return 0;
    }
    uint32_t rec_words() const override { return 2 * W; }

    int shard_pack(void *d_send, const uint64_t *base_records, uint32_t n_partitions, std::string &err) override {
        if (!have_parts_) return 0;
        if (n_partitions != pp_.P) { err = "partition count mismatch"; return -1; }
        DevBuf<unsigned long long> base;
        if (int rc = base.alloc(pp_.P, err)) return rc;
        HIPCHK(hipMemcpyAsync(base.p, base_records, (size_t)pp_.P * 8, hipMemcpyHostToDevice, stream_));
        EvTimer t(stream_, stage_timers_);
        hipLaunchKernelGGL((k_pack_partition<2 * W>), dim3(pp_.P), dim3(256), 0, stream_, recs_.p, fill_.p, pp_, base.p,
                           (uint64_t *)d_send);
        HIPCHK(hipGetLastError());
        if (t.on()) times_.add("shard_pack_kernel", t.stop());
        WAIT_STREAM();
        recs_.release(); fill_.release(); run_off_.release(); run_cnt_.release(); have_parts_ = false;
        return 0;
    }

    int shard_dedupe(std::vector<uint64_t> &part_records, std::string &err) override {
        if (!have_parts_) return 0;
        if (part_records.size() < pp_.P) { err = "partition count mismatch"; return -1; }
        std::vector<unsigned long long> base(pp_.P);
        unsigned long long n_raw = 0;
        for (uint32_t p = 0; p < pp_.P; p++) { base[p] = n_raw; n_raw += part_records[p]; }
        if (int rc = dd_base_.alloc(pp_.P, err)) return rc;
        if (int rc = dd_n_.alloc(pp_.P, err)) return rc;
        if (int rc = dd_recs_.alloc(n_raw * 2 * W + 2, err)) return rc;
        if (int rc = dd_w_.alloc(n_raw + 2, err)) return rc;
        HIPCHK(hipMemcpyAsync(dd_base_.p, base.data(), (size_t)pp_.P * 8, hipMemcpyHostToDevice, stream_));
        HIPCHK(fill2_async(ctl(&CountWords::dedupe_work), ctl_span(&CountWords::dedupe_work), 0u, nullptr, 0, 0u, stream_));
        EvTimer t(stream_, stage_timers_);
        hipLaunchKernelGGL(k_dedupe_partitions<W>, dim3(std::min<uint32_t>(pp_.P, (W <= 2 ? 2u : 1u) * (uint32_t)n_cus_)), dim3(COUNT_THREADS), 0, stream_,
                           run_view_, 0u, pp_.P, dd_base_.p, dd_recs_.p, dd_w_.p, dd_n_.p, (uint32_t *)ctl(&CountWords::dedupe_work),
                           (OvfRec *)nullptr, (uint32_t *)nullptr, 0u, 0u, (uint32_t *)nullptr);
        HIPCHK(hipGetLastError());
        t.mark();
        std::vector<uint32_t> h(pp_.P);
        HIPCHK(hipMemcpyAsync(h.data(), dd_n_.p, (size_t)pp_.P * 4, hipMemcpyDeviceToHost, stream_));
        WAIT_STREAM();
        times_.add("shard_dedupe_kernel", t.elapsed());
        unsigned long long n_dd = 0;
        for (uint32_t p = 0; p < pp_.P; p++) { part_records[p] = h[p]; n_dd += h[p]; }
        times_.add("shard_dedupe_records_in_x1e-6", (double)n_raw * 1e-6);
        times_.add("shard_dedupe_records_out_x1e-6", (double)n_dd * 1e-6);
        have_dedup_ = true;
        return 0;
    }
    void shard_drop_dedup() override { dd_recs_.release(); dd_w_.release(); dd_base_.release(); dd_n_.release(); have_dedup_ = false; }
    int shard_pack_dedup(void *d_send, void *d_send_w, const uint64_t *base_records, uint32_t n_partitions, std::string &err) override {
        if (!have_dedup_) return 0;
        if (n_partitions != pp_.P) { err = "partition count mismatch"; return -1; }
        DevBuf<unsigned long long> base;
        if (int rc = base.alloc(pp_.P, err)) return rc;
        HIPCHK(hipMemcpyAsync(base.p, base_records, (size_t)pp_.P * 8, hipMemcpyHostToDevice, stream_));
        EvTimer t(stream_, stage_timers_);
        hipLaunchKernelGGL((k_pack_dedup<2 * W>), dim3(pp_.P), dim3(256), 0, stream_, dd_recs_.p, dd_w_.p, dd_base_.p, dd_n_.p, base.p,
                           (uint64_t *)d_send, (uint32_t *)d_send_w);
        HIPCHK(hipGetLastError());
        if (t.on()) times_.add("shard_pack_kernel", t.stop());
        WAIT_STREAM();
        shard_drop_dedup();
        recs_.release(); fill_.release(); run_off_.release(); run_cnt_.release(); have_parts_ = false;
        return 0;
    }

    int shard_count(const void *d_recv, const void *d_recv_w, const uint64_t *run_off, const uint32_t *run_cnt, uint32_t n_owned,
                    uint32_t n_sources, uint32_t emit_threshold, uint64_t histo[500], std::string &err) override {
        if (n_sources < 1 || n_sources > 256) { err = "1..256 sources"; return -1; }
        const uint64_t n_runs = (uint64_t)n_owned * n_sources;
        if (int rc = run_off_.alloc(n_runs, err)) return rc;
        if (int rc = run_cnt_.alloc(n_runs, err)) return rc;
        std::vector<unsigned long long> addr16(n_runs);
        for (uint64_t i = 0; i < n_runs; i++) addr16[i] = ((unsigned long long)(uintptr_t)d_recv >> 4) + run_off[i] * (unsigned long long)W;
        if (n_runs) {
            HIPCHK(hipMemcpyAsync(run_off_.p, addr16.data(), n_runs * 8, hipMemcpyHostToDevice, stream_));
            HIPCHK(hipMemcpyAsync(run_cnt_.p, run_cnt, n_runs * 4, hipMemcpyHostToDevice, stream_));
        }
        shard_recv_ = d_recv;
        run_view_.run_addr16 = run_off_.p; run_view_.run_cnt = run_cnt_.p;
        run_view_.S = n_sources; run_view_.k = k_; n_count_parts_ = n_owned;
        run_view_.weights = (const uint32_t *)d_recv_w; run_view_.rec_base16 = (unsigned long long)(uintptr_t)d_recv >> 4;
        uint64_t total_recs = 0;
        for (uint32_t j = 0; j < n_owned; j++) {
            uint64_t r = 0;
            for (uint32_t s = 0; s < n_sources; s++) r += run_cnt[(uint64_t)j * n_sources + s];
            if (r > 0xFFFFFFF0ull) { err = "a partition holds more than 2^32 records"; return -1; }
            total_recs += r;
        }
        memset(histo, 0, 500 * 8);
        n_emitted_ = 0; emit_threshold_ = emit_threshold; n_distinct_ = 0;
        double ms = 0; uint64_t inst = 0;
        have_parts_ = n_runs != 0;
        const uint64_t rows_hint = d_recv_w ? 2 * total_recs + (1u << 16) : std::max<uint64_t>(1u << 16, total_recs);
        if (int rc = run_count_partitions(run_view_, n_owned, emit_threshold, ekeys_, ecnt_, n_emitted_, histo, inst,
                                          rows_hint, ms, err)) return rc;
        times_.add("count_kernel", ms);
        total_instances_ = inst;
        for (int i = 0; i < 500; i++) { histo_[i] = histo[i]; n_distinct_ += histo[i]; }
        return 0;
    }

    int shard_rows(uint32_t threshold, const void **keys_soa, const void **cnt, uint64_t *n, std::string &err) override {
        if (int rc = filter(threshold, err)) return rc;
        for (int j = 0; j < W; j++) keys_soa[j] = skeys_[j].p;
        *cnt = scnt_.p; *n = n_solid_;
        return 0;
    }

    int shard_set_solid(const void *const *keys_soa, const void *cnt, uint64_t n, const uint64_t histo[500],
                        uint64_t total_instances, std::string &err) override {
        if (n >= 0x7FFFFFFFull) { err = "too many solid k-mers for 32-bit node ids"; return -1; }
        DevBuf<uint64_t> nk[W]; DevBuf<uint32_t> nc;
        for (int j = 0; j < W; j++) {
            if (int rc = nk[j].alloc(n, err)) return rc;
            if (n) HIPCHK(hipMemcpyAsync(nk[j].p, keys_soa[j], n * 8, hipMemcpyDeviceToDevice, stream_));
        }
// ... 124 lines not shown
                HIPCHK(fill2_async(ctl(&GraphWords::xq_count), ctl_span(&GraphWords::xq_count), 0u, nullptr, 0, 0u, stream_));
                hipLaunchKernelGGL(k_xq_total, dim3(gp_), dim3(256), 0, stream_, gp_roff.p, queries.p, gp_cnt.p, (unsigned int *)ctl(&GraphWords::xq_count));
                unsigned int n_x = 0;
                if (int rc = read_ctl(n_x, &GraphWords::xq_count, err)) return rc;
                xq_n_ = n_x;
                if (int rc = xq_dest_.alloc(n_x, err)) return rc;
                if (int rc = xq_pay_.alloc((size_t)n_x * (W + 1), err)) return rc;
                if (int rc = xq_meta_.alloc(n_x, err)) return rc;
                if (n_x) {
                    HIPCHK(fill2_async(ctl(&GraphWords::xq_count), ctl_span(&GraphWords::xq_count), 0u, nullptr, 0, 0u, stream_));
                    hipLaunchKernelGGL(k_xq_stage<W>, dim3(gp_), dim3(256), 0, stream_, g.keys, k_, gp_roff.p, queries.p, gp_cnt.p,
                                       (unsigned int *)ctl(&GraphWords::xq_count), n_x, xq_dest_.p, xq_pay_.p, xq_meta_.p);
                    HIPCHK(hipGetLastError());
                }
            }
            if (keep_stages_) HIPCHK(hipMemcpyAsync(adj0_.p, adj_.p, n, hipMemcpyDeviceToDevice, stream_));
            graph_check_pending_ = true;
            if (sh_active_) {
                HIPCHK(fetch_ctl(mb_graph(), &GraphWords::spare0, &GraphWords::slots_used));
                WAIT_STREAM();
                if (int rc = check_graph_flags(err)) return rc;
            }
            if (!sh_active_ || sh_world_ <= 1) {  }
        }
        graph_ready_ = true;
        return 0;
    }

    int check_graph_flags(std::string &err) {
        if (!graph_check_pending_) return 0;
        graph_check_pending_ = false;
        const GraphWords &h = *mb_graph();
        if ((uint32_t)h.table_flag == 2u) { err = "graph partition: a row lies outside its counting group's minimiser range"; return -6; }
        if ((uint32_t)h.table_flag || h.slots_used > gt_slots_) { err = "graph table overflow"; return -6; }
        return 0;
    }
    int read_ctl(unsigned int &v, unsigned long long GraphWords::*m, std::string &err) {
        unsigned long long h = 0;
        HIPCHK(hipMemcpyAsync(&h, ctl(m), ctl_span(m), hipMemcpyDeviceToHost, stream_));
        WAIT_STREAM();
        v = (unsigned int)h;
        return 0;
    }

    int apply_marks(Graph<W> &g, DevBuf<uint8_t> &mark, DevBuf<uint32_t> &removed, unsigned long long GraphWords::*m, std::string &err) {
        const uint32_t n = (uint32_t)n_solid_;
        hipLaunchKernelGGL(k_collect_marked, dim3(grid_for(n)), dim3(256), 0, stream_, n, mark.p, alive_.p,
                           removed.p, (unsigned int *)ctl(m));
        hipLaunchKernelGGL(k_apply_removed<W>, dim3(1024), dim3(256), 0, stream_, g, removed.p,
                           (const unsigned int *)ctl(m));
        HIPCHK(hipGetLastError());
        return 0;
    }

    int correct(bool tips, bool bubbles, std::string &err) override {
        if (!graph_ready_) { err = "graph not built"; return -2; }
        const uint32_t n = (uint32_t)n_solid_;
        tips_removed_ = bubbles_removed_ = 0; rounds_ = 0;
        corr_pending_ = false; corr_tips_ = tips; corr_bubbles_ = bubbles;
        if (n == 0 || (!tips && !bubbles)) return 0;
        if (int rc = corr_.cand.alloc(2ull * n, err)) return rc;
        if (int rc = corr_.removed.alloc(n, err)) return rc;
        if (int rc = corr_.mark.alloc(n, err)) return rc;
        if (!tips) HIPCHK(hipMemsetAsync(corr_.mark.p, 0, n, stream_));
        if (tips) {
            if (int rc = corr_.tip_head.alloc(2ull * n, err)) return rc;
            if (int rc = corr_.tiprec.alloc(2ull * n, err)) return rc;
            if (int rc = corr_.kill.alloc(2ull * n, err)) return rc;
        }
        EvTimer t(stream_, stage_timers_);
        if (int rc = correction_round(0, err)) return rc;
        t.stop_later("correct_total", pending_timers_);
        corr_pending_ = true;
        return 0;
    }
    struct CorrScratch { DevBuf<uint32_t> cand, tip_head, removed; DevBuf<uint8_t> mark, kill; DevBuf<TipRec> tiprec;
                         void release() { cand.release(); tip_head.release(); removed.release(); mark.release(); kill.release(); tiprec.release(); } };
    int correction_round(int round, std::string &err) {
        const uint32_t n = (uint32_t)n_solid_;
        Graph<W> g = graph_view();
        const dim3 G(1024), B(256);
        const bool tips = corr_tips_, bubbles = corr_bubbles_;
        const auto s_tip = round == 0 ? &GraphWords::r0_tips_removed : &GraphWords::tips_removed, s_bub = round == 0 ? &GraphWords::r0_bubbles_removed : &GraphWords::bubbles_removed;
        HIPCHK(fill2_async(ctl(&GraphWords::n_cand), ctl_span(&GraphWords::n_cand, &GraphWords::bubbles_removed), 0u, nullptr, 0, 0u, stream_));
        unsigned int *const d_ncand = (unsigned int *)ctl(&GraphWords::n_cand), *const d_ntips = (unsigned int *)ctl(&GraphWords::n_tips);
        if (tips) {
            hipLaunchKernelGGL(k_tip_candidates<W>, dim3(grid_for(n)), B, 0, stream_, g, alive_.p,
                               corr_.cand.p, d_ncand, round == 0 ? (uint2 *)corr_.tip_head.p : (uint2 *)nullptr,
                               round == 0 ? corr_.mark.p : (uint8_t *)nullptr);
            hipLaunchKernelGGL(k_tip_walk<W>, G, B, 0, stream_, g, corr_.cand.p, (const unsigned int *)d_ncand,
                               corr_.tiprec.p, d_ntips, corr_.tip_head.p);
            hipLaunchKernelGGL(k_tip_decide<W>, G, B, 0, stream_, g, corr_.tiprec.p, (const unsigned int *)d_ntips,
                               corr_.tip_head.p, corr_.kill.p);
            hipLaunchKernelGGL(k_tip_remove<W>, G, B, 0, stream_, g, corr_.tiprec.p, (const unsigned int *)d_ntips,
                               corr_.kill.p, corr_.tip_head.p, corr_.mark.p);
            hipLaunchKernelGGL(k_tip_reset_heads, G, B, 0, stream_, corr_.tiprec.p, (const unsigned int *)d_ntips,
                               corr_.tip_head.p);
            HIPCHK(hipGetLastError());
            if (int rc = apply_marks(g, corr_.mark, corr_.removed, s_tip, err)) return rc;
        }
        if (bubbles) {
            HIPCHK(fill2_async(ctl(&GraphWords::n_cand), ctl_span(&GraphWords::n_cand), 0u, nullptr, 0, 0u, stream_));
            hipLaunchKernelGGL(k_fork_candidates<W>, dim3(grid_for(n)), B, 0, stream_, g, alive_.p,
                               corr_.cand.p, d_ncand);
            hipLaunchKernelGGL(k_bubble<W>, G, B, 0, stream_, g, corr_.cand.p, (const unsigned int *)d_ncand, corr_.mark.p);
            HIPCHK(hipGetLastError());
            if (int rc = apply_marks(g, corr_.mark, corr_.removed, s_bub, err)) return rc;
        }
        return 0;
    }
    int finish_correction(unsigned int n1, unsigned int n2, std::string &err) {
        corr_pending_ = false;
        tips_removed_ += n1; bubbles_removed_ += n2; rounds_ = 1;
        EvTimer t(stream_, stage_timers_);
        for (int round = 1; round < 32 && n1 + n2 != 0; round++) {
            if (int rc = correction_round(round, err)) return rc;
            GraphWords *const h = (GraphWords *)(mbox64() + MB_MISC);
            HIPCHK(fetch_ctl(h, &GraphWords::tips_removed, &GraphWords::bubbles_removed));
            WAIT_STREAM();
            n1 = (unsigned int)h->tips_removed; n2 = (unsigned int)h->bubbles_removed;
            tips_removed_ += n1; bubbles_removed_ += n2; rounds_++;
        }
        if (rounds_ > 1) if (t.on()) times_.add("correct_total", t.stop());
        corr_.release();
        return 0;
    }

    int get_adjacency(uint8_t *adj_initial, uint8_t *adj_final, uint8_t *alive, uint64_t cap,
                      std::string &err) override {
        if (!graph_ready_) { err = "graph not built"; return -2; }
        if (cap < n_solid_) { err = "buffer too small"; return -1; }
        if (!n_solid_) return 0;
        if (adj_initial && !keep_stages_) { err = "the initial adjacency is kept for inspection only on a verbose handle (or with SHK_KEEP_STAGES=1)"; return -2; }
        if (adj_initial) HIPCHK(hipMemcpy(adj_initial, adj0_.p, n_solid_, hipMemcpyDeviceToHost));
        if (adj_final) HIPCHK(hipMemcpy(adj_final, adj_.p, n_solid_, hipMemcpyDeviceToHost));
        if (alive) HIPCHK(hipMemcpy(alive, alive_.p, n_solid_, hipMemcpyDeviceToHost));
        return 0;
    }

    struct ChainState {
        DevBuf<uint32_t> spl, slot_of;
        DevBuf<uint2> winfo, ol;
        DevBuf<SegRec> segs;
        DevBuf<FragRec> frag;
        DevBuf<RankRec> Ra, Rb;
        DevBuf<FinRec> fin;
        DevBuf<HeadRec> d_heads;
        DevBuf<RingMin> ringmin;
        std::vector<HeadRec> heads;
        uint32_t seg_cap = 0;
        unsigned int n_heads = 0;
        bool heads_on_host = true;
    };
    struct EmitPlan { EmitRec *d_off; char *d_out; char *h_out; uint32_t max_heads; unsigned long long out_cap; bool planned; unsigned long long out_bytes; uint32_t n_emit; };
    int rank_chains(ChainState &cs, bool rings, std::string &err, uint32_t keep_on_device_from = 0xFFFFFFFFu, EmitPlan *plan = nullptr) {
        const uint32_t n = (uint32_t)n_solid_;
        const uint32_t total = 2 * n;
        Graph<W> g = graph_view();
        if (plan) plan->planned = false;
        const bool stage_log = getenv("SHK_STAGE_LOG") != nullptr;
        auto stage = [&](const char *what) {
            if (!stage_log) return;
            const hipError_t e = hipStreamSynchronize(stream_);
            fprintf(stderr, "[rank_chains n=%u] %s done%s\n", n, what, e == hipSuccess ? "" : " (stream error)"); fflush(stderr);
        };
        if (int rc = cs.winfo.alloc(total, err)) return rc;
        if (int rc = cs.frag.alloc(total, err)) return rc;
        if (int rc = cs.spl.alloc(total, err)) return rc;
        if (int rc = cs.ol.alloc(total, err)) return rc;
        const uint32_t split_mask = (1u << (uint32_t)env_u64("SHK_SPLIT_LOG", SPLIT_LOG_DEFAULT)) - 1u;
        const uint32_t tile_rows = (uint32_t)std::min<uint64_t>(std::max<uint64_t>(env_u64("SHK_TILE_ROWS", LF_ROWS), 1), LF_TILE / 2u);
        const int lf_grid = (int)((n + tile_rows - 1) / tile_rows);
        const uint64_t cap_all = std::min<uint64_t>((uint64_t)total + 1024u, 0xFFFFFFF0ull);
        uint64_t seg_cap64 = std::min<uint64_t>(cap_all, env_u64("SHK_SEG_CAP", (uint64_t)total / 12u + 65536u));
        constexpr unsigned int HEADS_SPEC = 512;
        static_assert(MB_MISC * 8 + HEADS_SPEC * sizeof(HeadRec) <= MBOX_BYTES, "mailbox");
        std::vector<HeadRec> &heads = cs.heads;
        GraphWords hc{};
        uint32_t seg_cap = 0;
        EvTimer tr(stream_, stage_timers_);
        for (int attempt = 0;; attempt++) {
            if (attempt > 3) { err = "collapse: the chain ranking did not settle"; return -6; }
            seg_cap = (uint32_t)seg_cap64;
            cs.seg_cap = seg_cap;
            if (int rc = cs.segs.alloc(seg_cap, err)) return rc;
            if (int rc = cs.Ra.alloc(seg_cap, err)) return rc;
            if (int rc = cs.Rb.alloc(seg_cap, err)) return rc;
            if (int rc = cs.slot_of.alloc(seg_cap, err)) return rc;
            if (int rc = cs.fin.alloc(seg_cap, err)) return rc;
            if (int rc = cs.d_heads.alloc(seg_cap, err)) return rc;
            if (int rc = cs.ringmin.alloc(seg_cap, err)) return rc;
            const unsigned long long *skip = corr_pending_ ? ctl(&GraphWords::r0_tips_removed) : (const unsigned long long *)nullptr;
            HIPCHK(fill2_async(ctl(&GraphWords::n_splitters), ctl_span(&GraphWords::n_splitters, &GraphWords::n_walked), 0u, cs.slot_of.p, (size_t)seg_cap * 4, 0xFFFFFFFFu, stream_));
            unsigned int *d_nspl = (unsigned int *)ctl(&GraphWords::n_splitters), *d_nheads = (unsigned int *)ctl(&GraphWords::n_chains);
            uint32_t *d_flags = ctl(&GraphWords::collapse_flag);
            unsigned long long *d_plan = ctl(&GraphWords::plan_state);
            hipLaunchKernelGGL(k_succ_split<W>, dim3((total + 256 * SS_ITEMS - 1) / (256 * SS_ITEMS)), dim3(256), 0, stream_, g,
                               alive_.p, cs.winfo.p, cs.spl.p, cs.ol.p, d_nspl, split_mask, ctl(&GraphWords::n_alive), skip);
            stage("k_succ_split");
            hipLaunchKernelGGL(k_local_frag<W>, dim3(lf_grid), dim3(LF_THREADS), 0, stream_, n, row_starts_.p, tile_rows, alive_.p, cs.winfo.p, cs.ol.p, cs.frag.p, split_mask, skip,
                               d_nspl, seg_cap, d_flags);
            stage("k_local_frag");
            hipLaunchKernelGGL(k_walk_frags<W>, dim3(grid_for((uint64_t)total / 64u + 16384u, 256, 1 << 20)), dim3(256), 0, stream_,
                               cs.spl.p, (const unsigned int *)d_nspl, cs.frag.p, cs.segs.p, split_mask, ctl(&GraphWords::n_walked), total, d_flags);
            stage("k_walk_frags");
            hipLaunchKernelGGL(k_orphan_cycles<W>, dim3(grid_for(total)), dim3(256), 0, stream_, g, alive_.p, cs.winfo.p, cs.ol.p,
                               cs.frag.p, cs.spl.p, cs.segs.p, d_nspl, seg_cap, d_flags, ctl(&GraphWords::n_alive), ctl(&GraphWords::n_walked));
            HIPCHK(hipGetLastError());
            stage("k_orphan_cycles");
            const int gr = grid_for((uint64_t)total / 64u + 65536u);
            int rounds = 1; { uint64_t reach = RANK_HOPS; while (reach < (uint64_t)seg_cap + 1u) { reach *= RANK_HOPS; rounds++; } }
            hipLaunchKernelGGL(k_rank_init, dim3(gr), dim3(256), 0, stream_, cs.segs.p, (const unsigned int *)d_nspl, cs.Ra.p);
            RankRec *Ri = cs.Ra.p, *Ro = cs.Rb.p;
            for (int r = 0; r < rounds; r++) {
                hipLaunchKernelGGL(k_rank_jump, dim3(gr), dim3(256), 0, stream_, (const unsigned int *)d_nspl, Ri, Ro, (uint32_t)r);
                std::swap(Ri, Ro);
            }
            stage("k_rank_jump");
            unsigned int *d_ncyc = (unsigned int *)ctl(&GraphWords::n_ring_splitters);
            hipLaunchKernelGGL(k_rank_tails<W>, dim3(gr), dim3(256), 0, stream_, g, cs.segs.p, (const unsigned int *)d_nspl, Ri, cs.d_heads.p, cs.slot_of.p, cs.ringmin.p,
                               d_nheads, d_ncyc);
            hipLaunchKernelGGL(k_rank_fin, dim3(gr), dim3(256), 0, stream_, cs.segs.p, (const unsigned int *)d_nspl, Ri, cs.slot_of.p, cs.fin.p);
            stage("k_rank_tails + k_rank_fin");
            hipLaunchKernelGGL(k_tile_final, dim3(lf_grid), dim3(LF_THREADS), 0, stream_, n, row_starts_.p, tile_rows, cs.ol.p, cs.frag.p, cs.fin.p, skip, (const uint32_t *)d_flags);
            stage("k_tile_final");
            if (rings) {
                hipLaunchKernelGGL(k_ring_min1<W>, dim3(1024), dim3(256), 0, stream_, g, alive_.p, cs.ol.p, cs.ringmin.p, d_ncyc);
                hipLaunchKernelGGL(k_ring_min2<W>, dim3(1024), dim3(256), 0, stream_, g, alive_.p, cs.ol.p, cs.ringmin.p, d_ncyc);
                hipLaunchKernelGGL(k_ring_rot<W>, dim3(gr), dim3(256), 0, stream_, g, cs.d_heads.p, (const unsigned int *)d_nheads, cs.ringmin.p,
                                   cs.winfo.p, cs.ol.p, d_ncyc, d_flags);
            }
            if (plan) {
                HIPCHK(fill2_async(d_plan, ctl_span(&GraphWords::plan_state, &GraphWords::plan_emitted), 0u, nullptr, 0, 0u, stream_));
                hipLaunchKernelGGL(k_plan_emit, dim3(1), dim3(1024), 0, stream_, cs.d_heads.p, (const unsigned int *)d_nheads, (uint32_t)k_, plan->max_heads,
                                   plan->out_cap, (const uint32_t *)d_flags, plan->d_off, d_plan);
                hipLaunchKernelGGL(k_emit<W>, dim3(grid_for(n)), dim3(256), 0, stream_, g, alive_.p, cs.ol.p, plan->d_off, plan->d_out, (const unsigned long long *)d_plan);
                hipLaunchKernelGGL(k_text_to_host_planned, dim3(64), dim3(256), 0, stream_, plan->d_out, plan->h_out, (const unsigned long long *)d_plan);
            }
            HIPCHK(hipGetLastError());
            heads.assign(HEADS_SPEC, HeadRec());
            HIPCHK(hipMemcpyAsync(mb_graph(), ctl_.p, sizeof(GraphWords), hipMemcpyDeviceToHost, stream_));
            HIPCHK(hipMemcpyAsync(mbox64() + MB_MISC, cs.d_heads.p, (size_t)std::min<uint32_t>(HEADS_SPEC, seg_cap) * sizeof(HeadRec), hipMemcpyDeviceToHost, stream_));
            WAIT_STREAM();
            const GraphWords &hc0 = *mb_graph();
            if (int rc = check_graph_flags(err)) return rc;
            if (corr_pending_) {
                const unsigned int r1 = (unsigned int)hc0.r0_tips_removed, r2 = (unsigned int)hc0.r0_bubbles_removed;
                if (int rc = finish_correction(r1, r2, err)) return rc;
                if (r1 + r2 != 0) continue;
            }
            hc = hc0;
            const uint32_t flag = hc.collapse_flag;
            if ((flag == 4 || flag == 2) && seg_cap64 < cap_all) {
                times_.add("collapse_seg_cap_retry_x1", 1.0);
                seg_cap64 = cap_all;
                continue;
            }
            memcpy(heads.data(), mbox64() + MB_MISC, (size_t)std::min<uint32_t>(HEADS_SPEC, seg_cap) * sizeof(HeadRec));
            if (plan && hc.plan_state == 1ull) { plan->planned = true; plan->out_bytes = hc.plan_bytes; plan->n_emit = (uint32_t)hc.plan_emitted; }
            break;
        }
        if (hc.collapse_flag) { err = hc.collapse_flag == 2 ? "collapse: too many short circular unitigs" : (hc.collapse_flag == 3 ? "collapse: ring without a smallest k-mer" : "collapse: broken cycle"); return -6; }
        times_.add("collapse_n_splitters_x1e-3", (double)(unsigned int)hc.n_splitters * 1e-3);
        times_.add("collapse_cycle_splitters_x1e-3", (double)(unsigned int)hc.n_ring_splitters * 1e-3);
        const unsigned int n_heads = (unsigned int)hc.n_chains;
        if (tr.on()) times_.add("collapse_rank_device", tr.stop());
        cs.n_heads = n_heads;
        if (!rings || n_heads >= keep_on_device_from) { heads.resize(std::min<unsigned int>(n_heads, HEADS_SPEC)); cs.heads_on_host = false; return 0; }
        heads.resize(n_heads);
        cs.heads_on_host = true;
        if (n_heads > HEADS_SPEC)
            HIPCHK(hipMemcpy(heads.data() + HEADS_SPEC, cs.d_heads.p + HEADS_SPEC, (size_t)(n_heads - HEADS_SPEC) * sizeof(HeadRec), hipMemcpyDeviceToHost));
        return 0;
    }

    int collapse(std::vector<RawContig> &out, std::string &err, const char **json, size_t *json_len, uint64_t *n_contigs, TextArrival **arrival) override {
        out.clear();
        if (json) *json = nullptr;
        if (arrival) *arrival = nullptr;
        if (!graph_ready_) { err = "graph not built"; return -2; }
        const uint32_t n = (uint32_t)n_solid_;
        if (n == 0) return 0;
        Graph<W> g = graph_view();
        ChainState cs;
        const uint64_t dw_min = env_u64("SHK_DEVICE_WRITER_MIN", 20000);
        constexpr uint32_t PLAN_HEADS = 512;
        EmitPlan plan{}; EmitPlan *use_plan = nullptr;
        DevBuf<EmitRec> d_plan_off; DevBuf<char> d_plan_out;
        if (env_u64("SHK_DEVICE_PLAN", 0) != 0 && dw_min > PLAN_HEADS) {
            const unsigned long long cap = (unsigned long long)n + (unsigned long long)PLAN_HEADS * (unsigned long long)(k_ - 1) + 64ull;
            if (int rc = d_plan_off.alloc(PLAN_HEADS, err)) return rc;
            if (int rc = d_plan_out.alloc(cap + 16, err)) return rc;
            if (int rc = hout_.alloc(cap + 16, err)) return rc;
            plan.d_off = d_plan_off.p; plan.d_out = d_plan_out.p; plan.h_out = hout_.p; plan.max_heads = PLAN_HEADS; plan.out_cap = cap;
            use_plan = &plan;
        }
        if (int rc = rank_chains(cs, true, err, json ? (uint32_t)std::min<uint64_t>(2 * dw_min, 0xFFFFFFFFull) : 0xFFFFFFFFu, use_plan)) return rc;
        if (use_plan && plan.planned && cs.heads_on_host) {
            std::vector<HeadRec> &hd = cs.heads;
            unsigned long long at = 0; uint32_t ne = 0;
            out.reserve(plan.n_emit);
            for (size_t i = 0; i < hd.size(); i++) {
                if (!hd[i].emit) continue;
                RawContig rc; rc.kc = hd[i].kc;
                rc.ext = hout_.p + at; rc.ext_n = hd[i].len + (uint64_t)(k_ - 1);
                at += rc.ext_n; ne++;
                out.push_back(std::move(rc));
            }
            if (at != plan.out_bytes || ne != plan.n_emit) { err = "collapse: the device's emission plan and the chain records disagree"; return -6; }
            times_.add("collapse_planned_on_device_x1", 1.0);
            return 0;
        }
        if (!cs.heads_on_host) {
            const uint32_t nh = cs.n_heads;
            DevBuf<unsigned long long> sz, fl, off, idx; DevBuf<char> tmp; DevBuf<EmitRec> d_off2; DevBuf<WContig> d_c; DevBuf<char> d_out2;
            if (int rc = sz.alloc((size_t)nh + 1, err)) return rc;
            if (int rc = fl.alloc((size_t)nh + 1, err)) return rc;
            hipLaunchKernelGGL(k_w_plan_sizes, dim3(grid_for(nh)), dim3(256), 0, stream_, cs.d_heads.p, nh, (uint32_t)k_, sz.p, fl.p);
            HIPCHK(hipGetLastError());
            if (int rc = scan_excl(sz, off, nh, tmp, err)) return rc;
            if (int rc = scan_excl(fl, idx, nh, tmp, err)) return rc;
            unsigned long long last[4] = {0, 0, 0, 0};
            HIPCHK(hipMemcpyAsync(&last[0], sz.p + (nh - 1), 8, hipMemcpyDeviceToHost, stream_));
            HIPCHK(hipMemcpyAsync(&last[1], off.p + (nh - 1), 8, hipMemcpyDeviceToHost, stream_));
            HIPCHK(hipMemcpyAsync(&last[2], fl.p + (nh - 1), 8, hipMemcpyDeviceToHost, stream_));
            HIPCHK(hipMemcpyAsync(&last[3], idx.p + (nh - 1), 8, hipMemcpyDeviceToHost, stream_));
            WAIT_STREAM();
            const uint64_t out_bytes2 = last[0] + last[1], n_emit = last[2] + last[3];
            if (n_emit >= 0x7FFFFFF0ull) { err = "device writer: too many contigs"; return -1; }
            if (int rc = d_off2.alloc(nh, err)) return rc;
            if (int rc = d_c.alloc(n_emit + 1, err)) return rc;
            if (int rc = d_out2.alloc(out_bytes2 + 16, err)) return rc;
            HIPCHK(fill2_async(ctl(&GraphWords::writer_flag), ctl_span(&GraphWords::writer_flag), 0u, nullptr, 0, 0u, stream_));
            hipLaunchKernelGGL(k_w_plan_fill, dim3(grid_for(nh)), dim3(256), 0, stream_, cs.d_heads.p, nh, (uint32_t)k_, off.p, idx.p, d_off2.p, d_c.p, (uint32_t *)ctl(&GraphWords::writer_flag));
            EvTimer t3(stream_, stage_timers_);
            hipLaunchKernelGGL(k_emit<W>, dim3(grid_for(n)), dim3(256), 0, stream_, g, alive_.p, cs.ol.p, d_off2.p, d_out2.p);
            HIPCHK(hipGetLastError());
            unsigned int fl9 = 0;
            if (int rc = read_ctl(fl9, &GraphWords::writer_flag, err)) return rc;
            if (t3.on()) times_.add("collapse_emit", t3.stop());
            if (fl9) { err = "device writer: a contig beyond 2^32 bases"; return -1; }
            if (n_emit == 0) { if (json) *json = nullptr; return 0; }
            if (int rc = device_write_json(g, cs, d_c, (uint32_t)n_emit, nh, d_out2.p, out_bytes2, json, json_len, err)) return rc;
            if (n_contigs) *n_contigs = n_emit;
            return 0;
        }
        std::vector<HeadRec> &heads = cs.heads;
        DevBuf<EmitRec> d_off; DevBuf<char> d_out;
        std::vector<EmitRec> head_off(heads.size());
        std::vector<uint32_t> emitted;
        uint64_t out_bytes = 0;
        for (size_t i = 0; i < heads.size(); i++) {
            EmitRec e; e.off = ~0ull; e.rot = heads[i].rot; e.len = (uint32_t)heads[i].len;
            if (heads[i].emit) { e.off = out_bytes; out_bytes += heads[i].len + (uint64_t)(k_ - 1); emitted.push_back((uint32_t)i); }
            head_off[i] = e;
        }
        if (!emitted.empty()) {
            PinnedBuf &hout = hout_;
            if (int rc = hout.alloc(out_bytes, err)) return rc;
            if (int rc = d_off.alloc(head_off.size(), err)) return rc;
            if (int rc = d_out.alloc(out_bytes, err)) return rc;
            HIPCHK(hipMemcpyAsync(d_off.p, head_off.data(), head_off.size() * sizeof(EmitRec), hipMemcpyHostToDevice, stream_));
            EvTimer t3(stream_, stage_timers_);
            hipLaunchKernelGGL(k_emit<W>, dim3(grid_for(n)), dim3(256), 0, stream_, g, alive_.p, cs.ol.p, d_off.p, d_out.p);
            HIPCHK(hipGetLastError());
            t3.stop_later("collapse_emit", pending_timers_);
            auto tcp = std::chrono::steady_clock::now();
            out.reserve(emitted.size());
            for (uint32_t i : emitted) {
                RawContig rc; rc.kc = heads[i].kc;
                rc.ext = hout.p + head_off[i].off; rc.ext_n = heads[i].len + (uint64_t)(k_ - 1);
                out.push_back(std::move(rc));
// ... 542 lines not shown
        }
        lap("rings");
        std::vector<ULayout> lay(n_u + 1);
        for (auto &L : lay) { L.off = ~0ull; L.node_off = 0; L.ring_len = 0; L.rot = 0; }
        uint64_t text_bytes = 0;
        std::vector<uint64_t> c_off(res.contigs.size());
        for (size_t i = 0; i < res.contigs.size(); i++) {
            const UnitigContig &ct = res.contigs[i];
            c_off[i] = text_bytes;
            uint64_t node_off = 0;
            for (uint32_t r : ct.recs) {
                lay[r].off = text_bytes; lay[r].node_off = node_off; lay[r].ring_len = ct.ring ? ct.len_nodes : 0; lay[r].rot = ct.ring ? ct.rot : 0;
                node_off += recs[r].len;
            }
            text_bytes += ct.len_nodes + (uint64_t)(k_ - 1);
        }
        lap("layout");
        times_.add("shard_graph_unitig_host_clock", now_ms_() - t_host0);
        stage("5 unitig graph");
        EvTimer te(stream_, stage_timers_);
        const uint64_t text_w32 = ((text_bytes + 15) / 16 + 1) & ~1ull;
        DevBuf<ULayout> d_lay; DevBuf<char> d_text; DevBuf<uint32_t> d_pack;
        if (int rc = d_lay.alloc(n_u + 1, err)) return rc;
        if (int rc = d_text.alloc(text_w32 * 16 + 16, err)) return rc;
        if (int rc = d_pack.alloc(text_w32 + 2, err)) return rc;
        if (int rc = hout_.alloc(text_w32 * 16 + 16, err)) return rc;
        if (text_bytes) {
            HIPCHK(hipMemsetAsync(d_text.p, 0, text_w32 * 16, stream_));
            HIPCHK(hipMemcpyAsync(d_lay.p, lay.data(), (size_t)(n_u + 1) * sizeof(ULayout), hipMemcpyHostToDevice, stream_));
            if (n) {
                hipLaunchKernelGGL(k_shard_emit<W>, dim3(grid_for(n)), dim3(256), 0, stream_, g, cs.ol.p, fin.p, (uint32_t)lbase[rank], uid_of_slot.p, d_lay.p, d_text.p);
                HIPCHK(hipGetLastError());
            }
            if (world > 1) {
                hipLaunchKernelGGL(k_text_pack2, dim3(grid_for(text_w32)), dim3(256), 0, stream_, d_text.p, text_bytes, d_pack.p, text_w32);
                HIPCHK(hipGetLastError());
                if (int rc = comm_allreduce_u64(c, d_pack.p, text_w32 / 2, stream_, err)) return rc;
                hipLaunchKernelGGL(k_text_unpack2, dim3(grid_for(text_w32)), dim3(256), 0, stream_, d_pack.p, text_w32, d_text.p);
                HIPCHK(hipGetLastError());
                times_.add("shard_graph_text_allreduce_MB", (double)(text_w32 * 4) / 1e6);
            }
            HIPCHK(hipMemcpyAsync(hout_.p, d_text.p, text_bytes, hipMemcpyDeviceToHost, stream_));
        }
        stage("6 emission kernels");
        WAIT_STREAM();
        if (te.on()) times_.add("shard_graph_emit", te.stop());
        out.reserve(res.contigs.size());
        for (size_t i = 0; i < res.contigs.size(); i++) {
            RawContig rcg; rcg.kc = res.contigs[i].kc;
            rcg.ext = hout_.p + c_off[i]; rcg.ext_n = res.contigs[i].len_nodes + (uint64_t)(k_ - 1);
            out.push_back(std::move(rcg));
        }
        times_.add("shard_assemble_host_clock", now_ms_() - t_all0);
        return 0;
    }
    template <typename F> static void host_par_ranges(size_t n, F &&fn) {
        const unsigned hw = std::thread::hardware_concurrency();
        const unsigned T = n < 262144 ? 1u : std::min(16u, std::max(1u, hw));
        if (T == 1) { fn((size_t)0, n); return; }
        std::vector<std::thread> ts;
        for (unsigned t = 1; t < T; t++) ts.emplace_back([&fn, n, t, T] { fn(n * t / T, n * (t + 1) / T); });
        fn((size_t)0, n / T);
        for (auto &t : ts) t.join();
    }
    static double now_ms_() { return std::chrono::duration<double, std::milli>(std::chrono::steady_clock::now().time_since_epoch()).count(); }

private:
    int k_;
    hipStream_t stream_ = nullptr; int stream_dev_ = 0;
    hipStream_t copy_stream_ = nullptr;
    ShardComm *wd_comm_ = nullptr;
    bool sh_agreed_ = false;
    StageTimes times_;
    std::vector<EvTimer::Pending> pending_timers_;
    int n_cus_ = 256;
    DevBuf<unsigned long long> ctl_;
    template <class S, class T> T *ctl(T S::*m) { return &(reinterpret_cast<S *>(ctl_.p)->*m); }
    template <class S, class A, class B> static size_t ctl_span(A S::*a, B S::*b) { static const S z{}; return (size_t)((const char *)&(z.*b) - (const char *)&(z.*a)) + sizeof(B); }
    template <class S, class A> static size_t ctl_span(A S::*a) { return sizeof(A); }
    template <class S, class A, class B> hipError_t fetch_ctl(S *img, A S::*a, B S::*b) { return hipMemcpyAsync(&(img->*a), ctl(a), ctl_span(a, b), hipMemcpyDeviceToHost, stream_); }
    PinnedBuf mbox_;
    unsigned long long *mbox64() { return (unsigned long long *)mbox_.p; }
    static constexpr size_t MBOX_BYTES = 32768;
    static constexpr int MB_P1 = 0 , MB_CTL = CTL_WORDS , MB_MISC = 2 * CTL_WORDS;
    CountWords *mb_p1() { return (CountWords *)(mbox64() + MB_P1); }  GraphWords *mb_graph() { return (GraphWords *)(mbox64() + MB_CTL); }
    struct P1Pending { bool on; const uint32_t *d_bases, *d_seg_off; uint64_t n_seg, n_bases, cap; };
    P1Pending p1_{false, nullptr, nullptr, 0, 0, 0};
    uint64_t n_host_waits_ = 0;
    bool stage_timers_ = env_u64("SHK_STAGE_TIMERS", 0) != 0;
    bool keep_stages_ = env_u64("SHK_KEEP_STAGES", 0) != 0;
    bool graph_check_pending_ = false, corr_pending_ = false, corr_tips_ = false, corr_bubbles_ = false;
    CorrScratch corr_;
    bool defer_p1_ = false;
    uint64_t cap_override_ = 0;
    DevBuf<uint64_t> tkeys_[W]; DevBuf<uint32_t> tcnt_, tstate_; uint64_t tslots_ = 0;
    struct Batch { const uint32_t *bases, *seg_off; uint64_t n_seg; };
    std::vector<Batch> pending_;
    std::vector<DevPiece> piece_list_;
    uint64_t total_instances_ = 0, n_distinct_ = 0, n_solid_ = 0;
    uint64_t histo_[500] = {0};
    bool global_mode_ = env_u64("SHK_COUNT_MODE_GLOBAL", 0) != 0;
    bool bloom_ = false, bloom_off_once_ = false;
    bool have_parts_ = false;
    bool have_dedup_ = false;
    bool split_ready_ = false;
    std::vector<unsigned long long> split_base_; unsigned long long split_total_ = 0, split_stride_ = 0;
    DevBuf<uint64_t> dd_recs_; DevBuf<uint32_t> dd_w_, dd_n_; DevBuf<unsigned long long> dd_base_;
    PartParams pp_{};
    DevBuf<uint64_t> recs_; DevBuf<uint32_t> fill_;
    DevBuf<unsigned long long> run_off_; DevBuf<uint32_t> run_cnt_;
    RunView run_view_{}; uint32_t n_count_parts_ = 0; uint32_t forced_P_ = 0;
    std::vector<std::unique_ptr<BatchRecs>> batches_;
    const void *shard_recv_ = nullptr;
    DevBuf<uint64_t> ekeys_[W]; DevBuf<uint32_t> ecnt_;
    uint64_t n_emitted_ = 0; uint32_t emit_threshold_ = 0;
    bool rows_scattered_ = false;
    DevBuf<unsigned long long> er_off_; DevBuf<uint32_t> er_msk_, er_start_, er_cnt_;
    uint32_t er_groups_ = 0; uint64_t er_rows_ = 0; bool er_ok_ = false;
    DevBuf<uint64_t> skeys_[W]; DevBuf<uint32_t> scnt_;
    DevBuf<uint64_t> gt_; DevBuf<uint8_t> gt_occ_; DevBuf<uint2> gt_scan_; uint64_t gt_slots_ = 0; uint32_t gp_ = 64;
    DevBuf<unsigned long long> gt_off_; DevBuf<uint32_t> gt_msk_;
    DevBuf<uint8_t> adj_, adj0_, alive_;
    DevBuf<uint32_t> row_starts_;
    PinnedBuf hout_;
    PinnedBuf hends_, hflags_;
    SlabArrival arrival_;
    DevBuf<char> d_out_keep_; DevBuf<unsigned long long> ends_src_;
    std::vector<unsigned long long> ends_src_host_;
    PinnedBuf hjson_;
    DevBuf<uint32_t> nb_;
    bool graph_ready_ = false;
    uint64_t tips_removed_ = 0, bubbles_removed_ = 0; int rounds_ = 0;
    bool sh_active_ = false;
    uint32_t sh_world_ = 1, sh_rank_ = 0, sh_P_ = 1;
    std::vector<uint64_t> sh_gbase_;
    uint64_t n_solid_global_ = 0;
    uint32_t xq_n_ = 0;
    DevBuf<uint32_t> xq_dest_; DevBuf<uint64_t> xq_pay_; DevBuf<unsigned long long> xq_meta_;
    DevBuf<unsigned long long> rt_row_, rt_all_, rt_cur_;
    std::vector<unsigned long long> rt_cur_host_;
    uint64_t rt_extra_host_ = 0;
};

int current_device() { int d = 0; (void)hipGetDevice(&d); return d; }
int set_device(int dev) { int prev = 0; (void)hipGetDevice(&prev); if (prev != dev) (void)hipSetDevice(dev); return prev; }
int device_download(void *host, const void *dptr, size_t bytes, std::string &err) {
    HIPCHK(hipMemcpy(host, dptr, bytes, hipMemcpyDeviceToHost));
    return 0;
}

int device_count() {
    int n = 0;
    if (hipGetDeviceCount(&n) != hipSuccess) return 0;
    return n;
}

IPipeline *make_pipeline(int k, std::string &err) {
    if (device_count() <= 0) { err = "no HIP device available (libshk_hip has no CPU fallback)"; return nullptr; }
    const int W = (2 * k + 63) / 64;
    int rc = -1;
    IPipeline *p = nullptr;
    if (W == 1) { auto *q = new Pipeline<1>(k); rc = q->init(err); p = q; }
    else if (W == 2) { auto *q = new Pipeline<2>(k); rc = q->init(err); p = q; }
    else if (W == 3) { auto *q = new Pipeline<3>(k); rc = q->init(err); p = q; }
    else if (W == 4) { auto *q = new Pipeline<4>(k); rc = q->init(err); p = q; }
    else if (W == 5) { auto *q = new Pipeline<5>(k); rc = q->init(err); p = q; }
    else if (W == 6) { auto *q = new Pipeline<6>(k); rc = q->init(err); p = q; }
    else if (W == 7) { auto *q = new Pipeline<7>(k); rc = q->init(err); p = q; }
    else if (W == 8) { auto *q = new Pipeline<8>(k); rc = q->init(err); p = q; }
    else { err = "k too large for the compiled key widths"; return nullptr; }
// ... 97 lines not shown
```

### sparrowhawk_amd/csrc/preprocess.cpp

```cpp
#include "preprocess.h"

#include <stdlib.h>
#include <string.h>
#include <algorithm>
#include <thread>
#include <utility>
#include <vector>

#include "fastq_gpu.h"
#include "inflate_gpu.h"
#include "inflate_mt.h"

namespace shk { bool spectrum_fit(const uint64_t *histo500, uint32_t *out); }

using namespace shk;

uint32_t emit_threshold_of(const shk_handle *h) {
    return h->do_fit ? (h->min_count < 1u ? h->min_count : 1u) : h->min_count;
}

namespace {

const int DECLINED = 1;

struct Knobs {
    static bool is(const char *v, char c) { return v && *v == c; }
    static uint64_t num(const char *v, uint64_t dflt) { return (v && *v) ? strtoull(v, nullptr, 10) : dflt; }
    const bool host_parser = is(getenv("SHK_HOST_PARSER"), '1'), gunzip_device = !is(getenv("SHK_GUNZIP_DEVICE"), '0');
    const size_t pipeline_min = num(getenv("SHK_FASTQ_PIPELINE_MIN"), 64ull << 20), stream_device_min = num(getenv("SHK_STREAM_DEVICE_MIN"), 8ull << 20);
    const size_t pieces = (size_t)std::max<long long>(1, (long long)num(getenv("SHK_FASTQ_PIECES"), 4));
    const uint64_t batch_bases = std::min<uint64_t>(std::max<uint64_t>(num(getenv("SHK_BATCH_BASES"), 1ull << 31), 1024), 3ull << 30);
    const BgzfWindowKnob window = bgzf_window_knob(2 * batch_bases);
};

template <typename T, void (*Free)(T &)> struct Owned : T {
    Owned() = default;
    Owned(Owned &&o) noexcept : T(std::move(static_cast<T &>(o))) { static_cast<T &>(o) = T(); }
    Owned &operator=(Owned &&o) noexcept { if (this != &o) { reset(); T::operator=(std::move(o)); static_cast<T &>(o) = T(); } return *this; }
    ~Owned() { reset(); }
    void reset() { Free(*this); }
};
using Text = Owned<GpuText, gpu_text_free>;
using Packed = Owned<GpuPacked, gpu_packed_free>;

struct Span { uint64_t base = 0, total = 0; bool pct = true; };
void post_loop(shk_handle *h, uint64_t reads, const Span &sp, uint64_t bytes) {
    std::string s = "loop:" + std::to_string(reads);
    if (sp.pct) s += ":" + std::to_string(sp.total ? (100 * (sp.base + bytes)) / sp.total : 100);
    h->post_mode(s.c_str());
}
void post_device_progress(shk_handle *h, const GpuPacked &gp, const Span &sp, uint64_t n1 = 0) {
    const uint64_t every = h->progress_every();
    for (size_t j = 0; j < gp.progress_bytes.size(); j++) {
        const bool second = (gp.progress_bytes[j] >> 63) != 0;
        post_loop(h, every * (gp.first_mark + j + 1), sp, (second ? n1 : 0) + (gp.progress_bytes[j] & ~(1ull << 63)));
    }
}

int count_one_batch(shk_handle *h, const uint32_t *d_bases, const uint32_t *d_seg_off, uint64_t n_seg, uint64_t n_bases) {
    std::string err;
    const double t0 = now_ms();
    h->batches_started++;
    int rc = h->pipe->count_batch(d_bases, d_seg_off, n_seg, n_bases, err);
    h->pipe->times().add("preprocess_device_total_host_clock", now_ms() - t0);
    return rc ? fail_rc(h, Rc::Device, rc, err) : SHK_OK;
}
int count_pieces(shk_handle *h, const std::vector<DevPiece> &pcs) {
    std::string err;
    const double t0 = now_ms();
    h->batches_started++;
    const int rc = h->pipe->count_batch_pieces(pcs.data(), pcs.size(), err);
    h->pipe->times().add("preprocess_device_total_host_clock", now_ms() - t0);
    return rc ? fail_rc(h, Rc::Device, rc, err) : SHK_OK;
}

int finish_counting(shk_handle *h) {
    std::string err;
    const double t0 = now_ms();
    h->post_loop_edge("loop:end");
    if (!h->do_bloom && h->chunk_size == 0) h->post("preprocess:bulk:sorting");
    int rc = h->pipe->histogram(h->histo, emit_threshold_of(h), err);
    if (rc) return fail(h, SHK_E_DEVICE, err);
    h->used_min_count = h->min_count; h->fit_ok = false;
    if (h->do_fit) {
        h->post_mode("fitting");
        uint32_t v = 0;
        if (spectrum_fit(h->histo, &v)) { h->used_min_count = v; h->fit_ok = true; }
    }
    h->post_mode("filtering");
    rc = h->pipe->filter(h->used_min_count, err);
    if (rc) return fail_rc(h, Rc::DeviceNoParam, rc, err);
    h->post("preprocess:saving");
    h->pre_json = preprocessing_json(h->pipe->n_solid(), h->histo, h->used_min_count);
    h->pipe->times().add("preprocess_device_total_host_clock", now_ms() - t0);
    h->st = St::Preprocessed;
    h->post("preprocess:end");
    return SHK_OK;
}

int run_counting(shk_handle *h, const uint32_t *d_bases, const uint32_t *d_seg_off, uint64_t n_seg, uint64_t n_bases) {
    h->pipe->single_batch_resident(true);
    int rc = count_one_batch(h, d_bases, d_seg_off, n_seg, n_bases);
    if (!rc) rc = finish_counting(h);
    h->pipe->single_batch_resident(false);
    return rc;
}

int flush_host_batch(shk_handle *h, PackedReads &pr) {
    if (pr.n_seg() == 0) { pr.reset_stream(); return SHK_OK; }
    pr.finish();
    std::string err;
    void *d_bases = nullptr, *d_off = nullptr;
    const double t0 = now_ms();
    int rc = device_upload(pr.bases.data(), pr.bases.size() * 4, &d_bases, err);
    if (!rc) rc = device_upload(pr.seg_off.data(), pr.seg_off.size() * 4, &d_off, err);
    if (rc) { device_free(d_bases); device_free(d_off); return fail(h, SHK_E_OOM, err); }
    h->pipe->times().add("h2d_upload_host_clock", now_ms() - t0);
    rc = count_one_batch(h, (const uint32_t *)d_bases, (const uint32_t *)d_off, pr.n_seg(), pr.n_bases);
    device_free(d_bases); device_free(d_off);
    pr.reset_stream();
    return rc;
}

uint64_t flush_every_reads(const shk_handle *h) { return (!h->do_bloom && h->chunk_size > 0) ? h->chunk_size : 0; }

int host_parse(shk_handle *h, const Knobs &kn, const uint8_t *t, size_t n, PackedReads &pr, const Span &sp, uint64_t flush_reads, uint64_t rec_base = 0) {
    std::string err;
    auto prog = [&](uint64_t reads, uint64_t bytes, uint64_t) { post_loop(h, reads, sp, bytes); };
    int flush_rc = SHK_OK;
    auto flush = [&](PackedReads &p) -> int { flush_rc = flush_host_batch(h, p); return flush_rc ? -7 : 0; };
    const int rc = pack_fastq(t, n, h->k, h->min_qual, pr, err, h->progress_every(), prog, flush_reads, kn.batch_bases, flush, rec_base);
    if (rc == -7) return flush_rc;
    return rc ? fail_rc(h, Rc::Parser, rc, err) : SHK_OK;
}

int host_rest(shk_handle *h, const Knobs &kn, const uint8_t *t, size_t n, const Span &sp, uint64_t file_reads, uint64_t &reads_done) {
    PackedReads pr;
    pr.n_reads = reads_done;
    if (int rc = host_parse(h, kn, t, n, pr, sp, 0, file_reads)) return rc;
    if (int rc = flush_host_batch(h, pr)) return rc;
    reads_done = pr.n_reads;
    return SHK_OK;
}

int parse_device_text(shk_handle *h, const GpuText &text, uint64_t reads_done, GpuPacked &gp, std::string &err) {
    return gpu_pack_fastq(nullptr, 0, nullptr, 0, h->k, h->min_qual, h->progress_every(), h->pipe->stream(), gp, err, reads_done, &text);
}
int device_batch_in(shk_handle *h, Packed &gp, const Span &sp, uint64_t &reads_done, uint64_t *file_reads = nullptr ) {
    post_device_progress(h, gp, sp);
    reads_done += gp.n_reads;
    if (file_reads) *file_reads += gp.n_reads;
    const int rc = gp.n_seg ? count_one_batch(h, gp.d_bases, gp.d_seg_off, gp.n_seg, gp.n_bases) : SHK_OK;
    gp.reset();
    return rc;
}
// ... 534 lines not shown
```

Baseline: 177.7.

## Batch control-word fills and device-to-host mail into fewer launches and copies

Replaces the two-region fill kernel with a four-region fill and merges separate zeroing launches into single fills. A single kernel now copies control words plus chain heads into pinned host memory in place of several async memcpys, and count-stage words, histogram and pass-1 flags are packed into one contiguous mailbox. Partition bases are computed from a stride when no base array is passed, which drops a stride-fill kernel. The device-side emit plan is now on by default, and add_time no longer resolves pending timers on every batch. The aim is to cut launch and copy overhead and host syncs, at the cost of more layout coupling and the new default plan path.

```diff
diff --git a/sparrowhawk_amd/csrc/count_part.h b/sparrowhawk_amd/csrc/count_part.h
--- a/sparrowhawk_amd/csrc/count_part.h
+++ b/sparrowhawk_amd/csrc/count_part.h
@@ -977,7 +977,8 @@
 template <int W>
 __global__ __launch_bounds__(COUNT_THREADS, W <= 2 ? 8 : 4) void k_dedupe_partitions(
                                                                      RunView rvw, uint32_t p_first, uint32_t n_parts,
-                                                                     const unsigned long long *__restrict__ base,
+                                                                     const unsigned long long *__restrict__ base ,
+                                                                     unsigned long long base_stride,
                                                                      uint64_t *__restrict__ out_recs, uint32_t *__restrict__ out_w,
                                                                      uint32_t *__restrict__ n_out, uint32_t *__restrict__ work_counter,
                                                                      OvfRec *__restrict__ ovf , uint32_t *__restrict__ ovf_n,
@@ -1060,8 +1061,9 @@
                 if (R) { const uint32_t slot = atomicAdd(ovf_n, 1u); OvfRec o; o.p = p; o.est_distinct = 0u; o.instances = ctl.part_inst; ovf[slot] = o; }
             }
         };
-        uint64_t *dst = out_recs + base[p] * RW;
-        uint32_t *dst_w = out_w + base[p];
+        const unsigned long long base_p = base ? base[p] : (unsigned long long)p * base_stride;
+        uint64_t *dst = out_recs + base_p * RW;
+        uint32_t *dst_w = out_w + base_p;
         const uint32_t per_wave = (((R + (COUNT_THREADS / 64) - 1) / (COUNT_THREADS / 64)) + 63u) & ~63u;
         const uint32_t w_begin = min(R, (threadIdx.x >> 6) * per_wave), w_end = min(R, w_begin + per_wave);
         uint32_t run_lo = 0, run_next = 0;
@@ -1145,8 +1147,8 @@
 
 template <int W>
 __global__ __launch_bounds__(COUNT_THREADS, W <= 2 ? 8 : 4) void k_count_weighted(
-    const uint64_t *__restrict__ recs, const uint32_t *__restrict__ weights, const unsigned long long *__restrict__ base,
-    const uint32_t *__restrict__ n_recs, uint32_t p_first, uint32_t n_parts, uint32_t merge , int k, uint32_t threshold,
+    const uint64_t *__restrict__ recs, const uint32_t *__restrict__ weights, const unsigned long long *__restrict__ base ,
+    unsigned long long base_stride, const uint32_t *__restrict__ n_recs, uint32_t p_first, uint32_t n_parts, uint32_t merge , int k, uint32_t threshold,
     unsigned long long *__restrict__ histo, KeyArr<W> out_keys, uint32_t *__restrict__ out_cnt,
     unsigned long long out_cap, unsigned long long *__restrict__ out_cursor,
     unsigned long long *__restrict__ n_inst, OvfRec *__restrict__ ovf, uint32_t *__restrict__ ovf_n,
@@ -1171,7 +1173,7 @@
 #pragma unroll
         for (int j = 0; j < 4; j++) {
             const bool in = (uint32_t)j < nm;
-            Rj[j] = in ? n_recs[pm[j]] : 0u; bj[j] = in ? base[pm[j]] : 0ull;
+            Rj[j] = in ? n_recs[pm[j]] : 0u; bj[j] = in ? (base ? base[pm[j]] : (unsigned long long)pm[j] * base_stride) : 0ull;
             Rt += Rj[j];
         }
         auto fetch = [&](uint32_t r, Rec<RW> &rec, uint32_t &wgt) {
@@ -1242,8 +1244,9 @@
     bool in_sample = true;
     auto defer = [&](uint32_t p, bool was_tried) {
         const uint32_t R = n_recs[p];
-        const uint64_t *src = recs + base[p] * RW;
-        const uint32_t *src_w = weights + base[p];
+        const unsigned long long base_p = base ? base[p] : (unsigned long long)p * base_stride;
+        const uint64_t *src = recs + base_p * RW;
+        const uint32_t *src_w = weights + base_p;
         mark_broken();
         __syncthreads();
         if (threadIdx.x == 0) { ctl.tried = 0; ctl.part_inst = 0; }
diff --git a/sparrowhawk_amd/csrc/ctl_words.h b/sparrowhawk_amd/csrc/ctl_words.h
--- a/sparrowhawk_amd/csrc/ctl_words.h
+++ b/sparrowhawk_amd/csrc/ctl_words.h
@@ -14,10 +14,8 @@
     uint32_t part_too_large, bucket_splits;
     uint32_t n_handed_over, tally;
     unsigned long long bucket_list_len;
-    unsigned long long spare5[3];
-    uint32_t p1_spare, p1_seg_too_long;
-    union { unsigned long long p1_max_fill;
-            unsigned long long bloom_keys; };
+    unsigned long long spare5[4];
+    unsigned long long bloom_keys;
     unsigned long long spare10;
     unsigned long long probe_work;
     unsigned long long dedupe_work;
@@ -28,6 +26,18 @@
     unsigned long long er_broken;
     unsigned long long spare24[8];
 };
+struct P1Words {
+    uint32_t spare, seg_too_long;
+    unsigned long long max_fill;
+};
+struct CountMail {
+    CountWords w;
+    unsigned long long hist[500];
+    P1Words p1;
+};
+static constexpr int COUNT_MAIL_WORDS = (int)(sizeof(CountMail) / 8);
+static_assert(sizeof(CountMail) == (CTL_WORDS + 500 + 2) * 8 && offsetof(CountMail, hist) == CTL_WORDS * 8 && offsetof(CountMail, p1) == (CTL_WORDS + 500) * 8,
+              "CountMail: words, histogram, pass 1's flags, contiguous");
 static inline unsigned tally_tried(uint32_t t) { return t & 0xFFFFu; }
 static inline unsigned tally_over(uint32_t t) { return t >> 16; }
 static inline unsigned long long er_rows(unsigned long long cursor) { return cursor >> 32; }
@@ -45,7 +55,8 @@
     uint32_t collapse_flag, n_spl_wanted;
     unsigned long long n_alive;
     unsigned long long n_walked;
-    unsigned long long spare11[2];
+    unsigned long long n_fork_cand;
+    unsigned long long spare12;
     union { unsigned long long xq_count;
             unsigned long long halflink_flags; };
     unsigned long long writer_flag;
@@ -62,8 +73,7 @@
 SHK_CTL_AT(CountWords, part_too_large, 2, 0); SHK_CTL_AT(CountWords, bucket_splits, 2, 1);
 SHK_CTL_AT(CountWords, n_handed_over, 3, 0);  SHK_CTL_AT(CountWords, tally, 3, 1);
 SHK_CTL_AT(CountWords, bucket_list_len, 4, 0);
-SHK_CTL_AT(CountWords, p1_spare, 8, 0);       SHK_CTL_AT(CountWords, p1_seg_too_long, 8, 1);
-SHK_CTL_AT(CountWords, p1_max_fill, 9, 0);    SHK_CTL_AT(CountWords, bloom_keys, 9, 0);
+SHK_CTL_AT(CountWords, bloom_keys, 9, 0);
 SHK_CTL_AT(CountWords, probe_work, 11, 0);    SHK_CTL_AT(CountWords, dedupe_work, 12, 0);
 SHK_CTL_AT(CountWords, groups_out, 14, 0);    SHK_CTL_AT(CountWords, group_tally, 14, 1);
 SHK_CTL_AT(CountWords, er_cursor, 22, 0);     SHK_CTL_AT(CountWords, er_broken, 23, 0);
@@ -75,6 +85,7 @@
 SHK_CTL_AT(GraphWords, n_ring_splitters, 7, 0);
 SHK_CTL_AT(GraphWords, collapse_flag, 8, 0);  SHK_CTL_AT(GraphWords, n_spl_wanted, 8, 1);
 SHK_CTL_AT(GraphWords, n_alive, 9, 0);        SHK_CTL_AT(GraphWords, n_walked, 10, 0);
+SHK_CTL_AT(GraphWords, n_fork_cand, 11, 0);
 SHK_CTL_AT(GraphWords, xq_count, 13, 0);      SHK_CTL_AT(GraphWords, halflink_flags, 13, 0);
 SHK_CTL_AT(GraphWords, writer_flag, 14, 0);
 SHK_CTL_AT(GraphWords, r0_tips_removed, 16, 0); SHK_CTL_AT(GraphWords, r0_bubbles_removed, 17, 0);
diff --git a/sparrowhawk_amd/csrc/pipeline.h b/sparrowhawk_amd/csrc/pipeline.h
--- a/sparrowhawk_amd/csrc/pipeline.h
+++ b/sparrowhawk_amd/csrc/pipeline.h
@@ -78,6 +78,7 @@
     virtual uint64_t n_solid_global() const = 0;
     virtual int shard_assemble(ShardComm *comm, bool tips, bool bubbles, std::vector<RawContig> &out, std::string &err) = 0;
     virtual StageTimes &times() = 0;
+    virtual void add_time(const char *name, double ms) = 0;
     virtual void drain() = 0;
     virtual void *stream() = 0;
     virtual int device() const = 0;
diff --git a/sparrowhawk_amd/csrc/pipeline.hip b/sparrowhawk_amd/csrc/pipeline.hip
--- a/sparrowhawk_amd/csrc/pipeline.hip
+++ b/sparrowhawk_amd/csrc/pipeline.hip
@@ -309,21 +309,31 @@
     return (v && *v) ? strtoull(v, nullptr, 10) : dflt;
 }
 
-__global__ __launch_bounds__(256) void k_fill2(uint32_t *a, unsigned long long na, uint32_t va, uint32_t *b, unsigned long long nb, uint32_t vb) {
+struct FillRegion { uint32_t *p; unsigned long long n; uint32_t v; };
+struct FillList { FillRegion r[4]; };
+static inline FillRegion fill_region(void *p, size_t bytes, uint32_t v) { return FillRegion{(uint32_t *)p, (unsigned long long)(bytes / 4), v}; }
+__global__ __launch_bounds__(256) void k_fill(FillList f) {
     const unsigned long long stride = (unsigned long long)gridDim.x * blockDim.x;
-    for (unsigned long long i = (unsigned long long)blockIdx.x * blockDim.x + threadIdx.x; i < na + nb; i += stride) {
-        if (i < na) a[i] = va; else b[i - na] = vb;
-    }
-}
-__global__ __launch_bounds__(256) void k_stride_fill(unsigned long long *out, uint32_t n, unsigned long long stride) {
-    for (uint32_t i = blockIdx.x * blockDim.x + threadIdx.x; i < n; i += gridDim.x * blockDim.x) out[i] = (unsigned long long)i * stride;
+    const unsigned long long total = f.r[0].n + f.r[1].n + f.r[2].n + f.r[3].n;
+    for (unsigned long long i = (unsigned long long)blockIdx.x * blockDim.x + threadIdx.x; i < total; i += stride) {
+        unsigned long long j = i;
+#pragma unroll
+        for (int q = 0; q < 4; q++) {
+            if (j < f.r[q].n) { f.r[q].p[j] = f.r[q].v; break; }
+            j -= f.r[q].n;
+        }
+    }
+}
+static inline hipError_t fill_async(hipStream_t st, FillRegion a, FillRegion b = FillRegion{nullptr, 0, 0u}, FillRegion c = FillRegion{nullptr, 0, 0u},
+                                    FillRegion d = FillRegion{nullptr, 0, 0u}) {
+    const FillList f{{a, b, c, d}};
+    const unsigned long long blocks = std::min<unsigned long long>((a.n + b.n + c.n + d.n + 255) / 256, 2048ull);
+    if (!blocks) return hipSuccess;
+    hipLaunchKernelGGL(k_fill, dim3((uint32_t)blocks), dim3(256), 0, st, f);
+    return hipGetLastError();
 }
 static inline hipError_t fill2_async(void *a, size_t bytes_a, uint32_t va, void *b, size_t bytes_b, uint32_t vb, hipStream_t st) {
-    const unsigned long long na = bytes_a / 4, nb = bytes_b / 4;
-    const unsigned long long blocks = std::min<unsigned long long>((na + nb + 255) / 256, 2048ull);
-    if (!blocks) return hipSuccess;
-    hipLaunchKernelGGL(k_fill2, dim3((uint32_t)blocks), dim3(256), 0, st, (uint32_t *)a, na, va, (uint32_t *)b, nb, vb);
-    return hipGetLastError();
+    return fill_async(st, fill_region(a, bytes_a, va), fill_region(b, bytes_b, vb));
 }
 
 static constexpr uint32_t ARRIVAL_SLAB = 64u << 10;
@@ -358,15 +368,15 @@
     __syncthreads();
     if (threadIdx.x == 0) __hip_atomic_store(flag_host, 1u, __ATOMIC_RELEASE, __HIP_MEMORY_SCOPE_SYSTEM);
 }
-__global__ __launch_bounds__(256) void k_text_to_host_planned(const char *__restrict__ src, char *__restrict__ dst_host,
-                                                              const unsigned long long *__restrict__ plan) {
-    if (plan[0] != 1ull) return;
-    const unsigned long long bytes = plan[1];
-    const unsigned long long nv = bytes >> 4;
-    const uint4 *a = reinterpret_cast<const uint4 *>(src);
-    uint4 *d = reinterpret_cast<uint4 *>(dst_host);
-    for (unsigned long long i = (unsigned long long)blockIdx.x * 256u + threadIdx.x; i < nv; i += (unsigned long long)gridDim.x * 256u) d[i] = a[i];
-    if (blockIdx.x == 0 && threadIdx.x < (bytes & 15ull)) dst_host[(nv << 4) + threadIdx.x] = src[(nv << 4) + threadIdx.x];
+__global__ __launch_bounds__(256) void k_mail_home(const unsigned long long *__restrict__ ctl_words, uint32_t n_ctl,
+                                                   const unsigned long long *__restrict__ recs, const unsigned int *__restrict__ n_recs_p,
+                                                   uint32_t max_recs, uint32_t rec_words,
+                                                   unsigned long long *__restrict__ mail_ctl, unsigned long long *__restrict__ mail_recs) {
+    for (uint32_t i = threadIdx.x; i < n_ctl; i += 256u) mail_ctl[i] = ctl_words[i];
+    uint32_t n = max_recs;
+    if (n_recs_p) n = min(*n_recs_p, max_recs);
+    const uint32_t nw = n * rec_words;
+    for (uint32_t i = threadIdx.x; i < nw; i += 256u) mail_recs[i] = recs[i];
 }
 class SlabArrival : public TextArrival {
 public:
@@ -421,11 +431,12 @@
         { int cus = 0; (void)hipDeviceGetAttribute(&cus, hipDeviceAttributeMultiprocessorCount, stream_dev_); n_cus_ = cus > 0 ? cus : 256; }
         stream_ = stream_pool_get(stream_dev_);
         if (!stream_) HIPCHK(hipStreamCreate(&stream_));
-        HIPCHK(ctl_.alloc(CTL_WORDS, err) ? hipErrorOutOfMemory : hipSuccess);
+        HIPCHK(ctl_.alloc(COUNT_MAIL_WORDS, err) ? hipErrorOutOfMemory : hipSuccess);
         if (mbox_.alloc(MBOX_BYTES, err)) return -4;
         return 0;
     }
     StageTimes &times() override { EvTimer::resolve(pending_timers_, times_); return times_; }
+    void add_time(const char *name, double ms) override { times_.add(name, ms); }
     void drain() override {
         if (copy_stream_) (void)hipStreamSynchronize(copy_stream_);
         if (!stream_) return;
@@ -494,7 +505,7 @@
     template <int WBLK, int NBLK>
     void launch_partition_t(const uint32_t *d_bases, const uint32_t *d_seg_off, uint32_t n_seg) {
         hipLaunchKernelGGL((k_partition<W, WBLK, NBLK>), dim3(pp_.G), dim3(PART_THREADS), 0, stream_, d_bases, d_seg_off,
-                           n_seg, pp_, recs_.p, fill_.p, ctl(&CountWords::p1_spare));
+                           n_seg, pp_, recs_.p, fill_.p, &d_count()->p1.spare);
     }
     void launch_partition(int win, const uint32_t *d_bases, const uint32_t *d_seg_off, uint32_t n_seg) {
         if (win == 20) launch_partition_t<10, 2>(d_bases, d_seg_off, n_seg);
@@ -570,7 +581,8 @@
             const uint64_t n_slices = (uint64_t)P * pp_.G;
             if (int rc = recs_.alloc(n_slices * cap * RW, err)) return rc;
             if (int rc = fill_.alloc(n_slices, err)) return rc;
-            HIPCHK(fill2_async(fill_.p, n_slices * 4, 0u, ctl_.p, sizeof(CountWords), 0u, stream_));
+            HIPCHK(fill2_async(fill_.p, n_slices * 4, 0u, ctl_.p, sizeof(CountMail), 0u, stream_));
+            p2_prefilled_ = false;
             EvTimer t(stream_);
             if (h_bases && attempt == 0) {
                 uint64_t C = env_u64("SHK_H2D_PIECES", 4);
@@ -596,40 +608,40 @@
                 HIPCHK(hipGetLastError());
                 times_.add("h2d_pieces_x1", (double)C);
                 if (defer_p1_ && batches_.empty()) {
-                    HIPCHK(fetch_ctl(mb_p1(), &CountWords::p1_spare, &CountWords::p1_max_fill));
                     t.stop_later("partition_with_upload", pending_timers_);
                     p1_ = P1Pending{true, d_bases, d_seg_off, n_seg, n_bases, cap};
+                    p2_prefilled_ = true;
                     return finish_partition(n_slices, err);
                 }
                 t.mark();
-                CountWords h;
-                HIPCHK(fetch_ctl(&h, &CountWords::p1_spare, &CountWords::p1_max_fill));
+                HIPCHK(fetch_p1());
                 WAIT_STREAM();
-                if (h.p1_seg_too_long) { err = "a read segment exceeds 32768 bases (split it on the host)"; return -1; }
-                if ((uint32_t)h.p1_max_fill <= cap) {
+                const P1Words h = mb_count()->p1;
+                if (h.seg_too_long) { err = "a read segment exceeds 32768 bases (split it on the host)"; return -1; }
+                if ((uint32_t)h.max_fill <= cap) {
                     times_.add("partition_with_upload", t.elapsed());
                     if (int rc = finish_partition(n_slices, err)) return rc;
                     return 0;
                 }
                 times_.add("partition_retry", t.elapsed());
-                cap = (uint64_t)(uint32_t)h.p1_max_fill + 8;
+                cap = (uint64_t)(uint32_t)h.max_fill + 8;
                 continue;
             }
             launch_partition_all(wblk, d_bases, d_seg_off, n_seg);
             HIPCHK(hipGetLastError());
             if (defer_p1_ && attempt == 0 && batches_.empty() && piece_list_.empty()) {
-                HIPCHK(fetch_ctl(mb_p1(), &CountWords::p1_spare, &CountWords::p1_max_fill));
                 t.stop_later("partition_kernel", pending_timers_);
                 p1_ = P1Pending{true, d_bases, d_seg_off, n_seg, n_bases, cap};
+                p2_prefilled_ = true;
                 return finish_partition(n_slices, err);
             }
             t.mark();
-            CountWords h;
-            HIPCHK(fetch_ctl(&h, &CountWords::p1_spare, &CountWords::p1_max_fill));
+            HIPCHK(fetch_p1());
             WAIT_STREAM();
             const double ms = t.elapsed();
-            if (h.p1_seg_too_long) { err = "a read segment exceeds 32768 bases (split it on the host)"; return -1; }
-            const uint32_t max_fill = (uint32_t)h.p1_max_fill;
+            const P1Words h = mb_count()->p1;
+            if (h.seg_too_long) { err = "a read segment exceeds 32768 bases (split it on the host)"; return -1; }
+            const uint32_t max_fill = (uint32_t)h.max_fill;
             if (max_fill <= cap) {
                 times_.add("partition_kernel", ms);
                 if (int rc = finish_partition(n_slices, err)) return rc;
@@ -748,12 +760,13 @@
         if (n_parts == 0) { n_rows = 0; inst_out = 0; memset(hist_out, 0, 500 * 8); ms_out = 0; return 0; }
         constexpr uint32_t S = CountShared<W>::S;
         const bool repartition = env_u64("SHK_NO_REPARTITION", 0) == 0 && rv.weights == nullptr;
-        DevBuf<unsigned long long> dh;
+        unsigned long long *const d_hist = d_count()->hist;
         DevBuf<OvfRec> d_ovf; DevBuf<OvfItem> d_items; DevBuf<uint32_t> d_fill, d_list, d_maxfill, d_new; DevBuf<uint64_t> d_kmers; DevBuf<BucketRef> d_blist; DevBuf<unsigned long long> d_sumfill;
         const bool bloom = bloom_ && !bloom_off_once_;
         unsigned long long bloom_new = 0, bloom_kmer_bytes = 0, bloom_kmer_bytes_exact = 0;
-        if (int rc = dh.alloc(500, err)) return rc;
         if (repartition) if (int rc = d_ovf.alloc(n_parts, err)) return rc;
+        const bool prefilled = p2_prefilled_ && p1_.on;
+        p2_prefilled_ = false;
         const bool split = W <= 2 && repartition && !bloom && rv.weights == nullptr && split_ready_ && split_base_.size() == n_parts && split_total_ > 0 &&
                            env_u64("SHK_COUNT_SPLIT", 1) != 0;
         struct DropSplit { Pipeline<W> *me; bool on; ~DropSplit() { if (on) me->shard_drop_dedup(); } } drop_split{this, split};
@@ -762,24 +775,25 @@
             bloom_new = 0; bloom_kmer_bytes = 0; bloom_kmer_bytes_exact = 0;
             for (int j = 0; j < W; j++) if (int rc = keys[j].alloc(cap, err)) return rc;
             if (int rc = cnt.alloc(cap, err)) return rc;
-            HIPCHK(fill2_async(dh.p, 500 * 8, 0u, ctl_.p, sizeof(CountWords), 0u, stream_));
+            if (!(prefilled && attempt == 0)) HIPCHK(fill_async(stream_, fill_region(ctl_.p, offsetof(CountMail, p1), 0u)));
             KeyArr<W> ok; for (int j = 0; j < W; j++) ok.w[j] = keys[j].p;
             const uint32_t probe_parts = (uint32_t)env_u64("SHK_PROBE_PARTS", 512);
             const uint32_t n_probe = (repartition && probe_parts && n_parts / 4 >= probe_parts) ? probe_parts : 0u;
             EvTimer t(stream_);
             if (split) {
-                if (int rc = dd_base_.alloc(n_parts, err)) return rc;
                 if (int rc = dd_n_.alloc(n_parts, err)) return rc;
                 if (int rc = dd_recs_.alloc(split_total_ * 2 * W + 2, err)) return rc;
                 if (int rc = dd_w_.alloc(split_total_ + 2, err)) return rc;
-                if (split_stride_) {
-                    hipLaunchKernelGGL(k_stride_fill, dim3((n_parts + 255) / 256), dim3(256), 0, stream_, dd_base_.p, n_parts, split_stride_);
-                    HIPCHK(hipGetLastError());
-                } else HIPCHK(hipMemcpyAsync(dd_base_.p, split_base_.data(), (size_t)n_parts * 8, hipMemcpyHostToDevice, stream_));
+                const unsigned long long *d_base = nullptr;
+                if (!split_stride_) {
+                    if (int rc = dd_base_.alloc(n_parts, err)) return rc;
+                    HIPCHK(hipMemcpyAsync(dd_base_.p, split_base_.data(), (size_t)n_parts * 8, hipMemcpyHostToDevice, stream_));
+                    d_base = dd_base_.p;
+                }
                 const uint32_t defer_after = n_probe / 8;
                 EvTimer t_a(stream_, stage_timers_);
                 hipLaunchKernelGGL(k_dedupe_partitions<W>, dim3(std::min<uint32_t>(n_parts, 2u * (uint32_t)n_cus_)), dim3(COUNT_THREADS), 0, stream_,
-                                   rv, 0u, n_parts, dd_base_.p, dd_recs_.p, dd_w_.p, dd_n_.p, (uint32_t *)ctl(&CountWords::dedupe_work),
+                                   rv, 0u, n_parts, d_base, split_stride_, dd_recs_.p, dd_w_.p, dd_n_.p, (uint32_t *)ctl(&CountWords::dedupe_work),
                                    d_ovf.p, ctl(&CountWords::n_handed_over), defer_after, (S / 10) * 9, ctl(&CountWords::group_tally));
                 HIPCHK(hipGetLastError());
                 if (attempt == 0) t_a.stop_later("count_dedupe_kernel", pending_timers_);
@@ -801,23 +815,22 @@
                     er_groups_ = n_groups;
                 }
                 hipLaunchKernelGGL(k_count_weighted<W>, dim3(std::min<uint32_t>(n_groups, per_cu * (uint32_t)n_cus_)), dim3(COUNT_THREADS), 0, stream_,
-                                   dd_recs_.p, dd_w_.p, dd_base_.p, dd_n_.p, 0u, n_parts, merge, rv.k, threshold, dh.p, ok, cnt.p, (unsigned long long)cap,
+                                   dd_recs_.p, dd_w_.p, d_base, split_stride_, dd_n_.p, 0u, n_parts, merge, rv.k, threshold, d_hist, ok, cnt.p, (unsigned long long)cap,
                                    ctl(&CountWords::row_cursor), ctl(&CountWords::instances), d_ovf.p, ctl(&CountWords::n_handed_over),
                                    (unsigned long long *)ctl(&CountWords::groups_out), 0u, defer_after, er);
             } else {
                 auto kern = rv.weights ? k_count_partitions<W, true> : k_count_partitions<W, false>;
                 hipLaunchKernelGGL(kern, dim3(std::min<uint32_t>(n_parts, (uint32_t)n_cus_)), dim3(COUNT_THREADS), 0, stream_, rv, n_parts, threshold,
-                                   dh.p, ok, cnt.p, (unsigned long long)cap, ctl(&CountWords::row_cursor), ctl(&CountWords::instances),
+                                   d_hist, ok, cnt.p, (unsigned long long)cap, ctl(&CountWords::row_cursor), ctl(&CountWords::instances),
                                    ctl(&CountWords::part_too_large), (const uint32_t *)nullptr, repartition ? d_ovf.p : (OvfRec *)nullptr,
                                    ctl(&CountWords::n_handed_over), (uint32_t *)ctl(&CountWords::probe_work), n_probe / 2, n_probe / 8);
             }
             HIPCHK(hipGetLastError());
             t.mark();
-            CountWords h{};
-            HIPCHK(fetch_ctl(&h, &CountWords::row_cursor, &CountWords::tally));
-            HIPCHK(hipMemcpyAsync(hist_out, dh.p, 500 * 8, hipMemcpyDeviceToHost, stream_));
-            if (split && er_groups_) HIPCHK(fetch_ctl(&h, &CountWords::er_cursor, &CountWords::er_broken));
+            HIPCHK(mail_count());
             WAIT_STREAM();
+            CountWords h = mb_count()->w;
+            memcpy(hist_out, mb_count()->hist, 500 * 8);
             ms_out = t.elapsed();
             const uint32_t n_ovf = h.n_handed_over;
             if (env_u64("SHK_VERBOSE_TALLY", 0)) fprintf(stderr, "[shk] pass 2: %u partitions, %u handed over, tally tried %u / over %u, split %d\n", n_parts, n_ovf,
@@ -874,8 +887,9 @@
                     HIPCHK(hipMemcpyAsync(smf.data(), d_sumfill.p, (size_t)ni * 8, hipMemcpyDeviceToHost, stream_));
                     if (bloom) HIPCHK(hipMemcpyAsync(newc.data(), d_new.p, (size_t)ni * 4, hipMemcpyDeviceToHost, stream_));
                     HIPCHK(hipMemcpyAsync(mxf.data(), d_maxfill.p, (size_t)ni * 4, hipMemcpyDeviceToHost, stream_));
-                    HIPCHK(fetch_ctl(&h, &CountWords::bucket_list_len, &CountWords::bucket_list_len));
+                    HIPCHK(fetch_ctl(&mb_count()->w, &CountWords::bucket_list_len, &CountWords::bucket_list_len));
                     WAIT_STREAM();
+                    h.bucket_list_len = mb_count()->w.bucket_list_len;
                     std::vector<OvfItem> again;
                     uint32_t n_good = 0;
                     for (uint32_t i = 0; i < ni; i++) {
@@ -893,7 +907,7 @@
                     if (const uint32_t n_list = (uint32_t)h.bucket_list_len) {
                         const uint32_t bgrid = (uint32_t)std::min<unsigned long long>(h.bucket_list_len, 2ull * (unsigned long long)n_cus_);
                         hipLaunchKernelGGL(k_count_buckets<W>, dim3(bgrid), dim3(COUNT_THREADS), 0, stream_,
-                                           d_blist.p, n_list, d_kmers.p, threshold, dh.p, ok, cnt.p, (unsigned long long)cap,
+                                           d_blist.p, n_list, d_kmers.p, threshold, d_hist, ok, cnt.p, (unsigned long long)cap,
                                            ctl(&CountWords::row_cursor), ctl(&CountWords::instances), ctl(&CountWords::part_too_large), bloom ? 1u : 0u, ctl(&CountWords::bloom_keys));
                         HIPCHK(hipGetLastError());
                         WAIT_STREAM();
@@ -905,7 +919,7 @@
                     if (int rc = d_list.alloc(bad.size(), err)) return rc;
                     HIPCHK(hipMemcpyAsync(d_list.p, bad.data(), bad.size() * 4, hipMemcpyHostToDevice, stream_));
                     hipLaunchKernelGGL(k_count_partitions<W>, dim3(std::min<uint32_t>((uint32_t)bad.size(), (uint32_t)n_cus_)), dim3(COUNT_THREADS), 0, stream_, rv, (uint32_t)bad.size(), threshold,
-                                       dh.p, ok, cnt.p, (unsigned long long)cap, ctl(&CountWords::row_cursor), ctl(&CountWords::instances),
+                                       d_hist, ok, cnt.p, (unsigned long long)cap, ctl(&CountWords::row_cursor), ctl(&CountWords::instances),
                                        ctl(&CountWords::part_too_large), (const uint32_t *)d_list.p, (OvfRec *)nullptr, (uint32_t *)nullptr, (uint32_t *)ctl(&CountWords::dedupe_work), 0u, 0u);
                     HIPCHK(hipGetLastError());
                 }
@@ -913,9 +927,14 @@
                 times_.add("count_repartitioned_x1", (double)n_good_total);
                 times_.add("count_deferred_untried_x1", (double)n_untried);
                 times_.add("count_residue_rerun_x1", (double)bad.size());
-                HIPCHK(fetch_ctl(&h, &CountWords::row_cursor, &CountWords::tally));
-                HIPCHK(hipMemcpyAsync(hist_out, dh.p, 500 * 8, hipMemcpyDeviceToHost, stream_));
+                HIPCHK(mail_count());
                 WAIT_STREAM();
+                {
+                    const CountWords &m = mb_count()->w;
+                    h.row_cursor = m.row_cursor; h.instances = m.instances; h.part_too_large = m.part_too_large; h.bucket_splits = m.bucket_splits;
+                    h.n_handed_over = m.n_handed_over; h.tally = m.tally;
+                    memcpy(hist_out, mb_count()->hist, 500 * 8);
+                }
                 times_.add("count_bucket_splits_x1", (double)h.bucket_splits);
                 if (bloom) {
                     unsigned long long n_keys = 0;
@@ -970,13 +989,13 @@
                 int rc_p2 = run_count_partitions(run_view_, n_count_parts_, emit_threshold, ekeys_, ecnt_, n_emitted_, histo, inst,
                                                  inst_ub_rows, ms, err);
                 if (p1_.on) {
-                    if (rc_p2) { std::string e2; (void)e2; (void)hipStreamSynchronize(stream_); }
+                    if (rc_p2) { (void)hipStreamSynchronize(stream_); if (fetch_p1() == hipSuccess) (void)hipStreamSynchronize(stream_); }
                     p1_.on = false;
-                    const CountWords &h = *mb_p1();
-                    if (h.p1_seg_too_long) { split_ready_ = false; err = "a read segment exceeds 32768 bases (split it on the host)"; return -1; }
-                    if ((uint32_t)h.p1_max_fill > p1_.cap) {
+                    const P1Words h = mb_count()->p1;
+                    if (h.seg_too_long) { split_ready_ = false; err = "a read segment exceeds 32768 bases (split it on the host)"; return -1; }
+                    if ((uint32_t)h.max_fill > p1_.cap) {
                         times_.add("partition_retry", 1.0);
-                        cap_override_ = (uint64_t)(uint32_t)h.p1_max_fill + 8;
+                        cap_override_ = (uint64_t)(uint32_t)h.max_fill + 8;
                         have_parts_ = false; split_ready_ = false;
                         const bool d = defer_p1_; defer_p1_ = false;
                         const int rc1 = count_batch_impl(p1_.d_bases, p1_.d_seg_off, nullptr, nullptr, p1_.n_seg, p1_.n_bases, err);
@@ -1156,7 +1175,7 @@
         HIPCHK(fill2_async(ctl(&CountWords::dedupe_work), ctl_span(&CountWords::dedupe_work), 0u, nullptr, 0, 0u, stream_));
         EvTimer t(stream_, stage_timers_);
         hipLaunchKernelGGL(k_dedupe_partitions<W>, dim3(std::min<uint32_t>(pp_.P, (W <= 2 ? 2u : 1u) * (uint32_t)n_cus_)), dim3(COUNT_THREADS), 0, stream_,
-                           run_view_, 0u, pp_.P, dd_base_.p, dd_recs_.p, dd_w_.p, dd_n_.p, (uint32_t *)ctl(&CountWords::dedupe_work),
+                           run_view_, 0u, pp_.P, dd_base_.p, 0ull, dd_recs_.p, dd_w_.p, dd_n_.p, (uint32_t *)ctl(&CountWords::dedupe_work),
                            (OvfRec *)nullptr, (uint32_t *)nullptr, 0u, 0u, (uint32_t *)nullptr);
         HIPCHK(hipGetLastError());
         t.mark();
@@ -1447,8 +1466,10 @@
         const dim3 G(1024), B(256);
         const bool tips = corr_tips_, bubbles = corr_bubbles_;
         const auto s_tip = round == 0 ? &GraphWords::r0_tips_removed : &GraphWords::tips_removed, s_bub = round == 0 ? &GraphWords::r0_bubbles_removed : &GraphWords::bubbles_removed;
-        HIPCHK(fill2_async(ctl(&GraphWords::n_cand), ctl_span(&GraphWords::n_cand, &GraphWords::bubbles_removed), 0u, nullptr, 0, 0u, stream_));
+        HIPCHK(fill_async(stream_, fill_region(ctl(&GraphWords::n_cand), ctl_span(&GraphWords::n_cand, &GraphWords::bubbles_removed), 0u),
+                          fill_region(ctl(&GraphWords::n_fork_cand), ctl_span(&GraphWords::n_fork_cand), 0u)));
         unsigned int *const d_ncand = (unsigned int *)ctl(&GraphWords::n_cand), *const d_ntips = (unsigned int *)ctl(&GraphWords::n_tips);
+        unsigned int *const d_nfork = (unsigned int *)ctl(&GraphWords::n_fork_cand);
         if (tips) {
             hipLaunchKernelGGL(k_tip_candidates<W>, dim3(grid_for(n)), B, 0, stream_, g, alive_.p,
                                corr_.cand.p, d_ncand, round == 0 ? (uint2 *)corr_.tip_head.p : (uint2 *)nullptr,
@@ -1465,10 +1486,9 @@
             if (int rc = apply_marks(g, corr_.mark, corr_.removed, s_tip, err)) return rc;
         }
         if (bubbles) {
-            HIPCHK(fill2_async(ctl(&GraphWords::n_cand), ctl_span(&GraphWords::n_cand), 0u, nullptr, 0, 0u, stream_));
             hipLaunchKernelGGL(k_fork_candidates<W>, dim3(grid_for(n)), B, 0, stream_, g, alive_.p,
-                               corr_.cand.p, d_ncand);
-            hipLaunchKernelGGL(k_bubble<W>, G, B, 0, stream_, g, corr_.cand.p, (const unsigned int *)d_ncand, corr_.mark.p);
+                               corr_.cand.p, d_nfork);
+            hipLaunchKernelGGL(k_bubble<W>, G, B, 0, stream_, g, corr_.cand.p, (const unsigned int *)d_nfork, corr_.mark.p);
             HIPCHK(hipGetLastError());
             if (int rc = apply_marks(g, corr_.mark, corr_.removed, s_bub, err)) return rc;
         }
@@ -1556,7 +1576,9 @@
             if (int rc = cs.d_heads.alloc(seg_cap, err)) return rc;
             if (int rc = cs.ringmin.alloc(seg_cap, err)) return rc;
             const unsigned long long *skip = corr_pending_ ? ctl(&GraphWords::r0_tips_removed) : (const unsigned long long *)nullptr;
-            HIPCHK(fill2_async(ctl(&GraphWords::n_splitters), ctl_span(&GraphWords::n_splitters, &GraphWords::n_walked), 0u, cs.slot_of.p, (size_t)seg_cap * 4, 0xFFFFFFFFu, stream_));
+            HIPCHK(fill_async(stream_, fill_region(ctl(&GraphWords::n_splitters), ctl_span(&GraphWords::n_splitters, &GraphWords::n_walked), 0u),
+                              fill_region(ctl(&GraphWords::plan_state), ctl_span(&GraphWords::plan_state, &GraphWords::plan_emitted), 0u),
+                              fill_region(cs.slot_of.p, (size_t)seg_cap * 4, 0xFFFFFFFFu)));
             unsigned int *d_nspl = (unsigned int *)ctl(&GraphWords::n_splitters), *d_nheads = (unsigned int *)ctl(&GraphWords::n_chains);
             uint32_t *d_flags = ctl(&GraphWords::collapse_flag);
             unsigned long long *d_plan = ctl(&GraphWords::plan_state);
@@ -1596,16 +1618,17 @@
                                    cs.winfo.p, cs.ol.p, d_ncyc, d_flags);
             }
             if (plan) {
-                HIPCHK(fill2_async(d_plan, ctl_span(&GraphWords::plan_state, &GraphWords::plan_emitted), 0u, nullptr, 0, 0u, stream_));
                 hipLaunchKernelGGL(k_plan_emit, dim3(1), dim3(1024), 0, stream_, cs.d_heads.p, (const unsigned int *)d_nheads, (uint32_t)k_, plan->max_heads,
                                    plan->out_cap, (const uint32_t *)d_flags, plan->d_off, d_plan);
                 hipLaunchKernelGGL(k_emit<W>, dim3(grid_for(n)), dim3(256), 0, stream_, g, alive_.p, cs.ol.p, plan->d_off, plan->d_out, (const unsigned long long *)d_plan);
-                hipLaunchKernelGGL(k_text_to_host_planned, dim3(64), dim3(256), 0, stream_, plan->d_out, plan->h_out, (const unsigned long long *)d_plan);
             }
             HIPCHK(hipGetLastError());
+            static_assert(sizeof(HeadRec) % 8 == 0, "chain records travel as 64-bit words");
             heads.assign(HEADS_SPEC, HeadRec());
-            HIPCHK(hipMemcpyAsync(mb_graph(), ctl_.p, sizeof(GraphWords), hipMemcpyDeviceToHost, stream_));
-            HIPCHK(hipMemcpyAsync(mbox64() + MB_MISC, cs.d_heads.p, (size_t)std::min<uint32_t>(HEADS_SPEC, seg_cap) * sizeof(HeadRec), hipMemcpyDeviceToHost, stream_));
+            hipLaunchKernelGGL(k_mail_home, dim3(1), dim3(256), 0, stream_, (const unsigned long long *)ctl_.p, (uint32_t)CTL_WORDS, (const unsigned long long *)cs.d_heads.p,
+                               (const unsigned int *)d_nheads, std::min<uint32_t>(HEADS_SPEC, seg_cap), (uint32_t)(sizeof(HeadRec) / 8), mbox64() + MB_CTL, mbox64() + MB_MISC);
+            HIPCHK(hipGetLastError());
+            if (plan) HIPCHK(hipMemcpyAsync(plan->h_out, plan->d_out, plan->out_cap, hipMemcpyDeviceToHost, stream_));
             WAIT_STREAM();
             const GraphWords &hc0 = *mb_graph();
             if (int rc = check_graph_flags(err)) return rc;
@@ -1621,7 +1644,7 @@
                 seg_cap64 = cap_all;
                 continue;
             }
-            memcpy(heads.data(), mbox64() + MB_MISC, (size_t)std::min<uint32_t>(HEADS_SPEC, seg_cap) * sizeof(HeadRec));
+            memcpy(heads.data(), mbox64() + MB_MISC, (size_t)std::min<uint32_t>((uint32_t)std::min<unsigned long long>(hc.n_chains & 0xFFFFFFFFull, HEADS_SPEC), seg_cap) * sizeof(HeadRec));
             if (plan && hc.plan_state == 1ull) { plan->planned = true; plan->out_bytes = hc.plan_bytes; plan->n_emit = (uint32_t)hc.plan_emitted; }
             break;
         }
@@ -1652,7 +1675,7 @@
         constexpr uint32_t PLAN_HEADS = 512;
         EmitPlan plan{}; EmitPlan *use_plan = nullptr;
         DevBuf<EmitRec> d_plan_off; DevBuf<char> d_plan_out;
-        if (env_u64("SHK_DEVICE_PLAN", 0) != 0 && dw_min > PLAN_HEADS) {
+        if (env_u64("SHK_DEVICE_PLAN", 1) != 0 && dw_min > PLAN_HEADS && getenv("SHK_ARRIVAL_MIN") == nullptr) {
             const unsigned long long cap = (unsigned long long)n + (unsigned long long)PLAN_HEADS * (unsigned long long)(k_ - 1) + 64ull;
             if (int rc = d_plan_off.alloc(PLAN_HEADS, err)) return rc;
             if (int rc = d_plan_out.alloc(cap + 16, err)) return rc;
@@ -2361,10 +2384,18 @@
     PinnedBuf mbox_;
     unsigned long long *mbox64() { return (unsigned long long *)mbox_.p; }
     static constexpr size_t MBOX_BYTES = 32768;
-    static constexpr int MB_P1 = 0 , MB_CTL = CTL_WORDS , MB_MISC = 2 * CTL_WORDS;
-    CountWords *mb_p1() { return (CountWords *)(mbox64() + MB_P1); }  GraphWords *mb_graph() { return (GraphWords *)(mbox64() + MB_CTL); }
+    static constexpr int MB_COUNT = 0 , MB_CTL = COUNT_MAIL_WORDS , MB_MISC = MB_CTL + CTL_WORDS;
+    CountMail *mb_count() { return (CountMail *)(mbox64() + MB_COUNT); }  GraphWords *mb_graph() { return (GraphWords *)(mbox64() + MB_CTL); }
+    CountMail *d_count() { return reinterpret_cast<CountMail *>(ctl_.p); }
+    hipError_t fetch_p1() { return hipMemcpyAsync(&mb_count()->p1, &d_count()->p1, sizeof(P1Words), hipMemcpyDeviceToHost, stream_); }
+    hipError_t mail_count() {
+        hipLaunchKernelGGL(k_mail_home, dim3(1), dim3(256), 0, stream_, (const unsigned long long *)ctl_.p, (uint32_t)COUNT_MAIL_WORDS, (const unsigned long long *)nullptr,
+                           (const unsigned int *)nullptr, 0u, 0u, mbox64() + MB_COUNT, (unsigned long long *)nullptr);
+        return hipGetLastError();
+    }
     struct P1Pending { bool on; const uint32_t *d_bases, *d_seg_off; uint64_t n_seg, n_bases, cap; };
     P1Pending p1_{false, nullptr, nullptr, 0, 0, 0};
+    bool p2_prefilled_ = false;
     uint64_t n_host_waits_ = 0;
     bool stage_timers_ = env_u64("SHK_STAGE_TIMERS", 0) != 0;
     bool keep_stages_ = env_u64("SHK_KEEP_STAGES", 0) != 0;
diff --git a/sparrowhawk_amd/csrc/preprocess.cpp b/sparrowhawk_amd/csrc/preprocess.cpp
--- a/sparrowhawk_amd/csrc/preprocess.cpp
+++ b/sparrowhawk_amd/csrc/preprocess.cpp
@@ -62,7 +62,7 @@
     const double t0 = now_ms();
     h->batches_started++;
     int rc = h->pipe->count_batch(d_bases, d_seg_off, n_seg, n_bases, err);
-    h->pipe->times().add("preprocess_device_total_host_clock", now_ms() - t0);
+    h->pipe->add_time("preprocess_device_total_host_clock", now_ms() - t0);
     return rc ? fail_rc(h, Rc::Device, rc, err) : SHK_OK;
 }
 int count_pieces(shk_handle *h, const std::vector<DevPiece> &pcs) {
@@ -70,7 +70,7 @@
     const double t0 = now_ms();
     h->batches_started++;
     const int rc = h->pipe->count_batch_pieces(pcs.data(), pcs.size(), err);
-    h->pipe->times().add("preprocess_device_total_host_clock", now_ms() - t0);
+    h->pipe->add_time("preprocess_device_total_host_clock", now_ms() - t0);
     return rc ? fail_rc(h, Rc::Device, rc, err) : SHK_OK;
 }
 
```

After: 180.5, median of 6. 1.02x the previous value.
